# ugonfor/DGQ

Hardware: AMD Instinct MI355X
Metric: UNet denoise steps/sec @ SD1.4 512^2 W4A8 g16 (higher is better)
Workload: dtype int8 (W4A8 MFMA, int32 accumulate; fp32 between layers); 1 GPU; SD v1.4 UNet W4A8 g=16 (time-aware, log2 softmax real-time δ, start-peak), DDIM 50-step schedule, 512x512 (64x64 latents), CFG pair per step per GPU; config_id=c2, prompts_per_gpu=1, batch_per_gpu=2, parallelism=replicas x1 (no collectives)

## Files before the change

### dgq_amd/_lib.py

```python
import ctypes
import os

import torch

_HERE = os.path.dirname(os.path.abspath(__file__))
LIB_PATH = os.environ.get("DGQ_HIP_LIB") or os.path.join(_HERE, "csrc", "libdgq_hip.so")

_vp, _i, _f, _i64 = ctypes.c_void_p, ctypes.c_int, ctypes.c_float, ctypes.c_int64
ABI_VERSION = 123

SIGNATURES = {
    "dgq_version": [],
    "dgq_quantize_weight": [_vp, _vp, _vp, _vp, _i, _i, _i, _vp, _vp],
    "dgq_pack_w4": [_vp, _i, _i, _vp, _i, _i, _vp, _vp],
    "dgq_unpack_w4": [_vp, _i, _i, _i, _vp, _vp],
    "dgq_pack_w8": [_vp, _i, _i, _vp, _i, _vp, _vp],
    "dgq_quant_act": [_vp, _i, _i, _i, _i, _i, _i, _i, _i, _i, _vp, _vp, _vp, _i, _i, _vp, _vp, _i, _i, _vp, _vp, _i,
                      _vp, _vp, _i, _vp, _vp, _f, _vp],
    "dgq_groupnorm_scale_shift": [_vp, _i, _i, _i, _i, _i, _f, _vp, _vp, _vp, _vp, _vp, _i, _vp],
    "dgq_quant_act_parts": [_i, _i],
    "dgq_gemm_wxa8": [_vp, _vp, _i, _i, _i, _vp, _i, _i, _i, _vp, _vp, _vp, _vp, _i, _f, _vp, _vp, _vp, _vp, _vp, _i, _i,
                      _vp, ctypes.c_size_t, _vp, _vp],
    "dgq_gemm_workspace_bytes": [_i, _i, _i],
    "dgq_gemm_plan_splits": [_i, _i, _i, _i, _i, ctypes.c_size_t],
    "dgq_gemm_act_fuses": [_i, _i, _i, _i, _i, _i, _i, _i, _i],
    "dgq_gemm_conv_act_fuses": [_i] * 14,
    "dgq_groupnorm_from_partials": [_vp, _i, _vp, _i, _i, _i, _i, _f, _vp, _vp, _vp, _vp, _vp],
    "dgq_fakequant_rows": [_vp, _vp, _i, _i, _i, _i, _i, _i, _vp, _vp, _i, _i, _vp],
    "dgq_max_f32": [_vp, _i64, _i, _i, _vp, _vp],
    "dgq_logquant_f32": [_vp, _vp, _i64, _i, _i, _vp, _i, _vp],
    "dgq_attention_f32": [_vp, _vp, _vp, _vp, _i, _i, _i, _i, _i, _f, _i, _i, _vp, _i, _vp, _vp, ctypes.c_size_t, _vp],
    "dgq_attention": [_vp, _vp, _vp, _vp, _i, _i, _i, _i, _i, _i, _f, _i, _i, _vp, _i, _vp, _vp, ctypes.c_size_t, _vp],
    "dgq_conv2d_f32w": [_vp, _i, _i, _i, _i, _i, _i, _i, _i, _i, _vp, _vp, _i, _vp, _i, _i, _vp, _vp, _i, _vp, _i, _vp, _vp],
    "dgq_conv2d_wq": [_vp, _i, _i, _i, _i, _i, _i, _i, _i, _i, _i, _vp, _i, _i, _vp, _vp, _vp, _i, _i, _vp, _i, _i, _vp],
    "dgq_attention_fuses_fakequant": [_i, _i],
    "dgq_attention_workspace_bytes": [_i, _i, _i, _i, _i],
    "dgq_attention_sync_timeouts": [],
    "dgq_minmax_rows_cols": [_vp, _i, _i, _i, _i64, _vp, _vp, _vp, _vp, _vp, _i, _vp],
    "dgq_linear_smallm_batch": [_vp, _i, _i, _i, _i64, _i, _i, _vp, _i, _vp],
    "dgq_quant_act_batch": [_i, _vp, _vp],
    "dgq_quant_act_variant": [_vp],
    "dgq_quant_act_conv_tile": [_i, _i, _i, _i, _i, _vp],
    "dgq_gemm_wxa8_batch": [_i, _vp, _vp],
    "dgq_adaround_soft_fwd": [_vp, _vp, _vp, _vp, _i, _i, _i, _vp, _vp],
    "dgq_adaround_soft_bwd": [_vp, _vp, _vp, _vp, _vp, _i, _i, _i, _vp, _vp],
    "dgq_adaround_reg_blocks": [_i64],
    "dgq_adaround_reg_fwd": [_vp, _i64, _f, _vp, _vp],
    "dgq_adaround_reg_bwd": [_vp, _i64, _f, _vp, _vp, _vp],
    "dgq_timestep_embedding": [_vp, _i, _i64, _i, _i, _vp, _i, _vp],
    "dgq_cfg_ddim_step": [_vp, _vp, _vp, _vp, _i, _i64, _i, _i, _i, _f, _f, _f, _f, _f, _vp],
}



class GemmExtra(ctypes.Structure):
    _fields_ = [("residual", _vp), ("ldr", _i), ("res_div", _i), ("res_dtype", _i), ("fq_mode", _i), ("fq_delta", _vp), ("fq_zp", _vp),
                ("fq_T", _i), ("fq_D", _i), ("fq_skip", _i), ("fq_qmax", _f), ("geglu", _i), ("gn_partial", _vp), ("conv", _vp), ("flush_coef", _vp), ("wfrag", _vp), ("act", _vp), ("y2", _vp), ("ldy2", _i)]


class GemmAct(ctypes.Structure):
    _fields_ = [("x", _vp), ("x_dtype", _i), ("ldx", _i), ("K", _i), ("kdst", _vp), ("czp", _vp), ("bits", _i),
                ("pre_scale", _vp), ("pre_shift", _vp), ("rows_per_image", _i), ("pre_act", _i),
                ("ln_gamma", _vp), ("ln_beta", _vp), ("ln_eps", _f),
                ("kpat", _vp), ("B", _i), ("H", _i), ("W", _i), ("kh", _i), ("kw", _i), ("stride", _i), ("pad", _i)]


class GemmConv(ctypes.Structure):
    _fields_ = [("codes_in", _vp), ("pixsum", _vp), ("fill", _vp), ("B", _i), ("H", _i), ("W", _i), ("C", _i), ("ldc", _i), ("kh", _i),
                ("kw", _i), ("stride", _i), ("pad", _i), ("Ho", _i), ("Wo", _i), ("zero_code", _f), ("pixsum_parts", _i)]


class SmallMProblem(ctypes.Structure):
    _fields_ = [("wpacked", _vp), ("alpha", _vp), ("zw", _vp), ("gamma", _vp), ("vn", _vp), ("mdelta", _vp), ("mzp", _vp),
                ("y", _vp), ("ldy", _i), ("N", _i), ("Kp", _i), ("w_bits", _i), ("a_bits", _i)]


class QuantActArgs(ctypes.Structure):
    _fields_ = [("x", _vp), ("x_dtype", _i), ("B", _i), ("H", _i), ("W", _i), ("C", _i), ("kh", _i), ("kw", _i), ("stride", _i),
                ("pad", _i), ("ksrc", _vp), ("koff", _vp), ("klds", _vp), ("kdst", _vp), ("Kp", _i), ("per_m", _i), ("delta", _vp), ("zp", _vp),
                ("L", _i), ("bits", _i), ("codes", _vp), ("rowsum", _vp), ("ksplits", _i), ("pre_scale", _vp), ("pre_shift", _vp),
                ("pre_act", _i), ("ln_gamma", _vp), ("ln_beta", _vp), ("ln_eps", _f), ("kpat", _vp), ("ups", _i)]


class GemmArgs(ctypes.Structure):
    _fields_ = [("codes", _vp), ("rowsum", _vp), ("rowsum_parts", _i), ("M", _i), ("Kp", _i), ("wpacked", _vp), ("w_bits", _i),
                ("N", _i), ("per_m", _i), ("cdelta", _vp), ("cflush", _vp), ("mdelta", _vp), ("mzp", _vp), ("L", _i),
                ("offset", _f), ("alpha", _vp), ("zw", _vp), ("gamma", _vp), ("vn", _vp), ("y", _vp), ("y_dtype", _i), ("ldy", _i),
                ("extra", _vp)]


class AttnFq(ctypes.Structure):
    _fields_ = [("mode", _i), ("skip", _i), ("bits", _i), ("delta", _vp), ("zero_point", _vp)]


_lib = None


def load():
    global _lib
    if _lib is None:
        if not os.path.exists(LIB_PATH):
            raise RuntimeError(
                "dgq_amd: %s not found — build it with `make -C dgq_amd/csrc` (or __graft_entry__.build()); "
                "there is no CPU fallback" % LIB_PATH)
        lib = ctypes.CDLL(LIB_PATH)
        for name, args in SIGNATURES.items():
            fn = getattr(lib, name)
            fn.argtypes = args
            fn.restype = ctypes.c_size_t if name.endswith("_workspace_bytes") else ctypes.c_int
        if lib.dgq_version() != ABI_VERSION:
            raise RuntimeError("dgq_amd: %s is ABI revision %d, this binding was written against %d (include/dgq_hip.h: "
                               "DGQ_ABI_VERSION) — rebuild with `make -C dgq_amd/csrc`" % (LIB_PATH, lib.dgq_version(), ABI_VERSION))
        lib.dgq_last_error.argtypes = []
        lib.dgq_last_error.restype = ctypes.c_char_p
        _lib = lib
    return _lib


def last_error():
    return load().dgq_last_error().decode()


def check(rc, what):
    if rc != 0:
        raise RuntimeError("%s failed (%d): %s" % (what, rc, last_error()))


DTYPE_CODE = {torch.float32: 0, torch.float16: 1, torch.bfloat16: 2}


def ptr(t):
    if t is None:
        return None
    assert t.is_cuda, "dgq_amd kernels need device tensors (no CPU path)"
    return ctypes.c_void_p(t.data_ptr())


def stream():
    return ctypes.c_void_p(torch.cuda.current_stream().cuda_stream)


def require_gpu():
    if not torch.cuda.is_available():
        raise RuntimeError("dgq_amd: no GPU visible — the quantized path runs only through the HIP kernels "
                           "(no CPU fallback)")
    load()
```

### dgq_amd/csrc/attn_bf16x3.hip

```cpp
#include "attn_bf16x3_dev.h"

DGQ_DIAG_BUFFER(attn)


template <int D, typename TIn, int QM, bool VINT>
__global__ __launch_bounds__(256) void attn3_prep_kernel(const TIn* __restrict__ k, const TIn* __restrict__ v,
                                                         unsigned char* __restrict__ planes, int B, int H, int S, int NT,
                                                         FqDesc fk, FqDesc fv, float* __restrict__ delta_reset, int n_reset,
                                                         const TIn* __restrict__ q, float* __restrict__ qfq, int T, FqDesc fqq) {
    using G = Geo<D, QM, VINT>;
    constexpr bool QI8 = QM == 1;
    static_assert(D % 8 == 0, "head_dim must be a multiple of 8");
    const int bh = blockIdx.y, b = bh / H, hd = bh - b * H;
    DGQ_DIAG_DECL
    DGQ_STAMP(0); DGQ_STAMP_REAL(1); DGQ_STAMP_WHERE(2);
#ifdef DGQ_DIAG
    dg.t[13] = 1;
#define DGQ_ATTN_PREP_DONE() do { DGQ_STAMP(9); DGQ_DIAG_DRAIN(); DGQ_STAMP(10); DGQ_STAMP_REAL(11); DGQ_DIAG_FLUSH(attn, 4, (threadIdx.x >> 6) + 32768, threadIdx.x & 63); } while (0)
#else
#define DGQ_ATTN_PREP_DONE() do {} while (0)
#endif
    if (QM == 2 && (int)blockIdx.x >= 2 * NT) {
        const int t0 = ((int)blockIdx.x - 2 * NT) * 32;
        constexpr int QC = D / 8;
        unsigned short* qb = reinterpret_cast<unsigned short*>(qfq);
        float* qtab = reinterpret_cast<float*>(qb + (size_t)B * T * H * D);
        const float off = 0.5f * (fqq.qmax + 1.0f);
        constexpr int QIT = (32 * QC + 255) / 256;
        float x[QIT][8];
#pragma unroll
        for (int it = 0; it < QIT; ++it) {
            const int i = threadIdx.x + 256 * it, r = i / QC, c8 = i - r * QC;
            if (i < 32 * QC && t0 + r < T) load8<TIn>(q + ((int64_t)(b * T + t0 + r) * H + hd) * D + 8 * c8, x[it]);
        }
#pragma unroll
        for (int it = 0; it < QIT; ++it) {
            const int i = threadIdx.x + 256 * it, r = i / QC, c8 = i - r * QC;
            const int t = t0 + r;
            if (i >= 32 * QC || t >= T) continue;
            const int64_t row = (int64_t)(b * T + t) * H + hd;
            unsigned w[4];
#pragma unroll
            for (int j = 0; j < 8; ++j) {
                const int idx = fqq.mode == 0 ? 0 : (fqq.mode == 1 ? t - fqq.skip : 8 * c8 + j);
                const float dl = fqq.delta[idx];
                const unsigned bits = bf16_bits(fq_code(x[it][j], dl, dgq_rcp(dl), fqq.zp[idx], fqq.qmax, off));
                if (j & 1) w[j >> 1] |= bits << 16; else w[j >> 1] = bits;
            }
            *reinterpret_cast<uint4*>(qb + row * D + 8 * c8) = make_uint4(w[0], w[1], w[2], w[3]);
            if (c8 == 0) {
                const int idx = fqq.mode == 0 ? 0 : t - fqq.skip;
                qtab[row * 2] = fqq.mode == 2 ? 1.0f : fqq.delta[idx];
                qtab[row * 2 + 1] = fqq.mode == 2 ? 1.0f : fqq.zp[idx] - off;
            }
        }
        DGQ_ATTN_PREP_DONE(); return;
    }
    if (QI8 && (int)blockIdx.x >= 2 * NT) {
        const int t = ((int)blockIdx.x - 2 * NT) * 32 + (threadIdx.x >> 3);
        const int part = threadIdx.x & 7;
        int8_t* qc = reinterpret_cast<int8_t*>(qfq);
        float* qtab = reinterpret_cast<float*>(reinterpret_cast<unsigned char*>(qfq) + (size_t)B * T * H * G::DP32);
        if (t < T) {
            const int64_t row = (int64_t)(b * T + t) * H + hd;
            const int idx = fqq.mode == 0 ? 0 : t - fqq.skip;
            const float dl = fqq.delta[idx], z = fqq.zp[idx], inv = dgq_rcp(dl);
            const float off = 0.5f * (fqq.qmax + 1.0f);
            const float zc = z - off;
            const TIn* k0 = k + ((int64_t)(b * S) * H + hd) * D;
            float csum = 0.0f, sp = 0.0f;
            for (int c8 = part; c8 < G::DP32 / 8; c8 += 8) {
                float x[8] = {0.f, 0.f, 0.f, 0.f, 0.f, 0.f, 0.f, 0.f};
                unsigned w0 = 0, w1 = 0;
                if (8 * c8 < D) {
                    load8<TIn>(q + row * D + 8 * c8, x);
                    float kk[8] = {0.f, 0.f, 0.f, 0.f, 0.f, 0.f, 0.f, 0.f};
                    if (fk.skip > 0) load8<TIn>(k0 + 8 * c8, kk);
#pragma unroll
                    for (int j = 0; j < 8; ++j) {
                        const float c = fq_code(x[j], dl, inv, z, fqq.qmax, off);
                        csum += c;
                        sp += (c - zc) * kk[j];
                        const unsigned byte = ((unsigned)(int)c) & 0xFFu;
                        if (j < 4) w0 |= byte << (8 * j); else w1 |= byte << (8 * (j - 4));
                    }
                }
                *reinterpret_cast<uint2*>(qc + row * G::DP32 + 8 * c8) = make_uint2(w0, w1);
            }
#pragma unroll
            for (int o = 4; o > 0; o >>= 1) {
                csum += __shfl_xor(csum, o, 64);
                sp += __shfl_xor(sp, o, 64);
            }
            if (part == 0) *reinterpret_cast<float4*>(qtab + row * 4) = make_float4(dl, zc, csum - (float)D * zc, sp);
        }
        DGQ_ATTN_PREP_DONE(); return;
    }
    if ((int)blockIdx.x >= 2 * NT) {
        const int t0 = ((int)blockIdx.x - 2 * NT) * 32;
        constexpr int QC = D / 8;
        for (int i = threadIdx.x; i < 32 * QC; i += 256) {
            const int r = i / QC, c8 = i - r * QC;
            const int t = t0 + r;
            if (t >= T) continue;
            const int64_t o = ((int64_t)(b * T + t) * H + hd) * D + 8 * c8;
            float x[8];
            load8<TIn>(q + o, x);
            fq_apply8(fqq, x, t, 8 * c8);
            *reinterpret_cast<float4*>(qfq + o) = make_float4(x[0], x[1], x[2], x[3]);
            *reinterpret_cast<float4*>(qfq + o + 4) = make_float4(x[4], x[5], x[6], x[7]);
        }
        DGQ_ATTN_PREP_DONE(); return;
    }
    const bool do_k = (int)blockIdx.x < NT;
    const int tile = do_k ? (int)blockIdx.x : (int)blockIdx.x - NT;
    const int s0 = tile * KT;
    if (delta_reset && blockIdx.x == 0 && bh == 0)
        for (int i = threadIdx.x; i < n_reset; i += 256) delta_reset[i] = 0.0f;
    const int64_t kbase = ((int64_t)(b * S) * H + hd) * D, vbase = kbase;
    const int64_t HD = (int64_t)H * D;
    unsigned short* kimg = reinterpret_cast<unsigned short*>(planes + ((int64_t)bh * NT + tile) * G::IMG_BYTES);
    unsigned short* vimg = kimg + G::K_ELEMS;
    const TypedLd<TIn> ld{};
    if (do_k) prep_k_tile<D, QM, VINT>(ld, k, kbase, HD, S, s0, fk, fqq, kimg, threadIdx.x);
    else prep_v_tile<D, QM, VINT>(ld, v, vbase, HD, S, s0, fv, vimg, threadIdx.x);
    DGQ_ATTN_PREP_DONE();
}

template <int D, int NW, int QM, int TPS = 1>
__global__ __launch_bounds__(64 * NW) void attn3_stats_kernel(AttnParams p) {
    using G = Geo<D, QM>;
    constexpr bool QI8 = G::QI8, KS = QM == 3;
    constexpr int ST = TPS > 1 ? 3 : G::STATS_STAGES, NP = G::K_PIECES, TB = NP * 1024, SB = TPS * TB;
    extern __shared__ __attribute__((aligned(16))) unsigned char lds8[];
    const int tid = threadIdx.x, lane = tid & 63, wid = tid >> 6, h32 = lane >> 5;
    DGQ_DIAG_DECL
    DGQ_STAMP(0); DGQ_STAMP_REAL(1); DGQ_STAMP_WHERE(2);
#ifdef DGQ_DIAG
    dg.t[13] = 2;
#endif
    int bx, bh;
    attn_block_coords(p.xcd, bx, bh);
    const int b = bh / p.H, hd = bh - b * p.H;
    const int t = bx * (32 * NW) + wid * 32 + (lane & 31);
    const int tq = min(t, p.T - 1);
    const unsigned char* img_lane = p.planes + (int64_t)bh * p.NT * p.img_bytes + lane * 16;
    const uint32_t lds_base = (uint32_t)(uintptr_t)(lptr_t)lds8;
    const int nsp = gridDim.z, i0 = (int)((long)p.NT * blockIdx.z / nsp), i1 = (int)((long)p.NT * (blockIdx.z + 1) / nsp);
#pragma unroll
    for (int i = 0; i < ST - 1; ++i)
#pragma unroll
        for (int j = 0; j < TPS; ++j)
            issue_image<NP, NW>(img_lane + (int64_t)min(i0 + TPS * i + j, i1 - 1) * p.img_bytes, lds_base + i * SB + j * TB, wid);
    bf16x8 qf[3][QI8 ? 1 : G::NKK];
    v4i qc[G::NK32];
    float4 qt = make_float4(1.0f, 0.0f, 0.0f, 0.0f);
    if constexpr (QI8) load_q_i8<D>(qc, qt, p, (int64_t)(b * p.T + tq) * p.H + hd, h32);
    else if constexpr (QM == 2) load_q1<D>(qf, reinterpret_cast<const unsigned short*>(p.q) + ((int64_t)(b * p.T + tq) * p.H + hd) * D, h32);
    else load_q<D>(qf, p.q + ((int64_t)(b * p.T + tq) * p.H + hd) * D, h32, p.fq[0], tq);
    if constexpr (QM == 2) {
        const float2 t2 = *reinterpret_cast<const float2*>(p.qtab + ((int64_t)(b * p.T + tq) * p.H + hd) * 2);
        qt.x = t2.x;
        qt.y = t2.y;
        if constexpr (G::FOLDZ) fold_zmul<D>(qf, qt.y, h32);
    }
    float inv_dk = 1.0f, cq = 0.0f, dk = 1.0f;
    if constexpr (KS) {
        dk = p.fq[1].delta[0];
        inv_dk = 1.0f / dk;
        cq = -(p.fq[1].zp[0] - 0.5f * (p.fq[1].qmax + 1.0f)) * qt.z;
    }
    const float sl2 = p.scale * LOG2E * qt.x * dk;
    float mraw = -INFINITY, l = 0.0f, m2raw = -INFINITY;
    DGQ_STAMP(3);
    wait_image<NP, TPS * (ST - 2), NW>(wid);
    __builtin_amdgcn_s_barrier();
    DGQ_STAMP(4);
    int stage = 0, istage = ST - 1;
    for (int ib = i0; ib < i1; ib += TPS) {
#pragma unroll
      for (int jt = 0; jt < TPS; ++jt)
        issue_image<NP, NW>(img_lane + (int64_t)min(ib + TPS * (ST - 1) + jt, i1 - 1) * p.img_bytes, lds_base + istage * SB + jt * TB, wid);
#pragma unroll
      for (int jt = 0; jt < TPS; ++jt) {
        const int i = ib + jt;
        const unsigned char* tile_lds = lds8 + stage * SB + jt * TB;
        const int s0 = i * KT;
        v16f acc;
        if constexpr (QI8) acc = score_tile_i8<D, KS>(tile_lds, qc, qt, lane, i == 0 && p.kskip > 0, inv_dk, cq);
        else if constexpr (QM == 2) acc = score_tile_q1<D>(reinterpret_cast<const unsigned short*>(tile_lds), qf, qt.y, lane);
        else acc = score_tile<D>(reinterpret_cast<const unsigned short*>(tile_lds), qf, lane);
        const bool edge = (s0 + KT > p.S) || (s0 < p.skip);
        float tmax = -INFINITY, tmax2 = -INFINITY;
        if (edge) {
#pragma unroll
            for (int r = 0; r < 16; ++r) {
                const int s = s0 + key_of(r, h32);
                if (s >= p.S) acc[r] = -INFINITY;
                tmax = fmaxf(tmax, acc[r]);
                if (s >= p.skip) tmax2 = fmaxf(tmax2, acc[r]);
            }
        } else {
#pragma unroll
            for (int r = 0; r < 16; ++r) tmax = fmaxf(tmax, acc[r]);
            tmax2 = tmax;
        }
        const float mn = fmaxf(mraw, tmax);
        const float nb = (mn == -INFINITY) ? 0.0f : -(mn * sl2);
        f2 part = {0.0f, 0.0f};
        const f2 sl2v = {sl2, sl2}, nbv = {nb, nb};
#pragma unroll
        for (int r = 0; r < 16; r += 2) {
            const f2 a = pk_fma(f2{acc[r], acc[r + 1]}, sl2v, nbv);
            part = pk_add(part, f2{__builtin_amdgcn_exp2f(a.x), __builtin_amdgcn_exp2f(a.y)});
        }
        l = l * __builtin_amdgcn_exp2f(fmaf(mraw, sl2, nb)) + (part.x + part.y);
        mraw = mn;
        m2raw = fmaxf(m2raw, tmax2);
      }
        wait_image<NP, TPS * (ST - 2), NW>(wid);
        __builtin_amdgcn_s_barrier();
        stage = (stage + 1 == ST) ? 0 : stage + 1;
        istage = (istage + 1 == ST) ? 0 : istage + 1;
    }
    asm volatile("s_waitcnt vmcnt(0)" ::: "memory");
    DGQ_STAMP(5);
    {
        const float mo = __shfl_xor(mraw, 32, 64), lo = __shfl_xor(l, 32, 64);
        const float mm = fmaxf(mraw, mo), nb = -(mm * sl2);
        l = l * __builtin_amdgcn_exp2f(fmaf(mraw, sl2, nb)) + lo * __builtin_amdgcn_exp2f(fmaf(mo, sl2, nb));
        mraw = mm;
        m2raw = fmaxf(m2raw, __shfl_xor(m2raw, 32, 64));
    }
    mraw += cq;
    m2raw += cq;
    const float m = mraw * sl2;
    if (nsp > 1) {
        if (t < p.T && h32 == 0)
            *reinterpret_cast<float4*>(p.stats_part + (((int64_t)blockIdx.z * p.B * p.H + bh) * p.T + t) * 4) = make_float4(m, l, m2raw * sl2, 0.0f);
        DGQ_STAMP(9); DGQ_DIAG_DRAIN(); DGQ_STAMP(10); DGQ_STAMP_REAL(11);
        DGQ_DIAG_FLUSH(attn, NW, wid + 16384, lane);
        return;
    }
    if (t < p.T && h32 == 0) {
        float* st = p.stats + ((int64_t)bh * p.T + t) * 2;
        st[0] = m;
        st[1] = l;
    }
    if (p.mode == 1) {
        float pm = (t < p.T) ? exp2f(m2raw * sl2 - m) / l : 0.0f;
#pragma unroll
        for (int o = 32; o > 0; o >>= 1) pm = fmaxf(pm, __shfl_xor(pm, o, 64));
        float* wmax = reinterpret_cast<float*>(lds8);
        __syncthreads();
        if (lane == 0) wmax[wid] = pm;
        __syncthreads();
        if (tid == 0) {
#pragma unroll
            for (int w = 1; w < NW; ++w) pm = fmaxf(pm, wmax[w]);
            const int slot = (blockIdx.x + gridDim.x * blockIdx.y) & (DELTA_SLOTS - 1);
            atomicMax(reinterpret_cast<int*>(p.delta) + slot, __float_as_int(pm));
        }
    }
    DGQ_STAMP(9); DGQ_DIAG_DRAIN(); DGQ_STAMP(10); DGQ_STAMP_REAL(11);
    DGQ_DIAG_FLUSH(attn, NW, wid + 16384, lane);
}

template <typename T>
__global__ __launch_bounds__(256) void attn3_add16_kernel(T* __restrict__ o, const float* __restrict__ part0, const float* __restrict__ part1, int64_t n4) {
    const int64_t i = (int64_t)blockIdx.x * 256 + threadIdx.x;
    if (i < n4) {
        const float4 a = reinterpret_cast<const float4*>(part0)[i], c = reinterpret_cast<const float4*>(part1)[i];
        T t[4] = {dgq_from_float<T>(a.x + c.x), dgq_from_float<T>(a.y + c.y), dgq_from_float<T>(a.z + c.z), dgq_from_float<T>(a.w + c.w)};
        reinterpret_cast<uint2*>(o)[i] = *reinterpret_cast<const uint2*>(t);
    }
}

__global__ __launch_bounds__(256) void attn3_add_kernel(float* __restrict__ o, const float* __restrict__ part, int64_t n4) {
    const int64_t i = (int64_t)blockIdx.x * 256 + threadIdx.x;
    if (i < n4) {
        float4 a = reinterpret_cast<float4*>(o)[i];
        const float4 c = reinterpret_cast<const float4*>(part)[i];
        a.x += c.x; a.y += c.y; a.z += c.z; a.w += c.w;
        reinterpret_cast<float4*>(o)[i] = a;
    }
}

__global__ __launch_bounds__(256) void attn3_merge_kernel(AttnParams p) {
    const int64_t row = (int64_t)blockIdx.x * 256 + threadIdx.x, rows = (int64_t)p.B * p.H * p.T;
    float pm = 0.0f;
    if (row < rows) {
        const float4 a = *reinterpret_cast<const float4*>(p.stats_part + row * 4);
        const float4 c = *reinterpret_cast<const float4*>(p.stats_part + (rows + row) * 4);
        const float m = fmaxf(a.x, c.x);
        const float l = a.y * exp2f(a.x - m) + c.y * exp2f(c.x - m);
        p.stats[row * 2] = m;
        p.stats[row * 2 + 1] = l;
        if (p.mode == 1) pm = exp2f(fmaxf(a.z, c.z) - m) / l;
    }
    if (p.mode == 1) {
#pragma unroll
        for (int o = 32; o > 0; o >>= 1) pm = fmaxf(pm, __shfl_xor(pm, o, 64));
        __shared__ float wmax[4];
        if ((threadIdx.x & 63) == 0) wmax[threadIdx.x >> 6] = pm;
        __syncthreads();
        if (threadIdx.x == 0) {
            pm = fmaxf(fmaxf(wmax[0], wmax[1]), fmaxf(wmax[2], wmax[3]));
            atomicMax(reinterpret_cast<int*>(p.delta) + (blockIdx.x & (DELTA_SLOTS - 1)), __float_as_int(pm));
        }
    }
}

template <int D, bool UNIFORM, int NW, int QM, bool VINT, int TPS = 1>
__global__ __launch_bounds__(64 * NW) void attn3_pv_kernel(AttnParams p) {
    using G = Geo<D, QM, VINT>;
    constexpr bool QI8 = G::QI8, KS = QM == 3;
    constexpr int ST = TPS > 1 ? 2 : G::PV_STAGES, NP = G::IMG_PIECES, TB = G::IMG_BYTES, SB = TPS * TB;
    extern __shared__ __attribute__((aligned(16))) unsigned char lds8[];
    const int tid = threadIdx.x, lane = tid & 63, wid = tid >> 6, h32 = lane >> 5;
    DGQ_DIAG_DECL
    DGQ_STAMP(0); DGQ_STAMP_REAL(1); DGQ_STAMP_WHERE(2);
#ifdef DGQ_DIAG
    dg.t[13] = 3;
#endif
    int bx, bh;
    attn_block_coords(p.xcd, bx, bh);
    const int b = bh / p.H, hd = bh - b * p.H;
    const int t = bx * (32 * NW) + wid * 32 + (lane & 31);
    const int tq = min(t, p.T - 1);
    const unsigned char* img_lane = p.planes + (int64_t)bh * p.NT * G::IMG_BYTES + lane * 16;
    const uint32_t lds_base = (uint32_t)(uintptr_t)(lptr_t)lds8;
    const int nsp = gridDim.z, i0 = (int)((long)p.NT * blockIdx.z / nsp), i1 = (int)((long)p.NT * (blockIdx.z + 1) / nsp);
#pragma unroll
    for (int i = 0; i < ST - 1; ++i)
#pragma unroll
        for (int j = 0; j < TPS; ++j)
            issue_image<NP, NW>(img_lane + (int64_t)min(i0 + TPS * i + j, i1 - 1) * G::IMG_BYTES, lds_base + i * SB + j * TB, wid);
    bf16x8 qf[3][QI8 ? 1 : G::NKK];
    v4i qc[G::NK32];
    float4 qt = make_float4(1.0f, 0.0f, 0.0f, 0.0f);
    if constexpr (QI8) load_q_i8<D>(qc, qt, p, (int64_t)(b * p.T + tq) * p.H + hd, h32);
    else if constexpr (QM == 2) load_q1<D>(qf, reinterpret_cast<const unsigned short*>(p.q) + ((int64_t)(b * p.T + tq) * p.H + hd) * D, h32);
    else load_q<D>(qf, p.q + ((int64_t)(b * p.T + tq) * p.H + hd) * D, h32, p.fq[0], tq);
    if constexpr (QM == 2) {
        const float2 t2 = *reinterpret_cast<const float2*>(p.qtab + ((int64_t)(b * p.T + tq) * p.H + hd) * 2);
        qt.x = t2.x;
        qt.y = t2.y;
        if constexpr (G::FOLDZ) fold_zmul<D>(qf, qt.y, h32);
    }
    float inv_dk = 1.0f, cq = 0.0f, dk = 1.0f;
    if constexpr (KS) {
        dk = p.fq[1].delta[0];
        inv_dk = 1.0f / dk;
        cq = -(p.fq[1].zp[0] - 0.5f * (p.fq[1].qmax + 1.0f)) * qt.z;
    }
    const float2 ml = *reinterpret_cast<const float2*>(p.stats + ((int64_t)bh * p.T + tq) * 2);
    const float l = ml.y;
    float delta;
    if (p.mode == 1) {
        delta = p.delta[lane];
#pragma unroll
        for (int o = 32; o > 0; o >>= 1) delta = fmaxf(delta, __shfl_xor(delta, o, 64));
    } else {
        delta = p.delta[0];
    }
    const float sl2 = p.scale * LOG2E * qt.x * dk;
    const float nsl2 = -sl2;
    const float m = ml.x - cq * sl2;
    const float a0 = m + log2f(l) + log2f(delta);
    const float inv_l = 1.0f / l;
    constexpr float MAGIC = 12582912.0f;
    constexpr int MAGIC_I = 0x4B400000;
    const int cmax_i = MAGIC_I + min((int)p.qmax, 127);
    float p_bypass = 0.0f;
    float psum = 0.0f;
    v16f oacc[G::NDT];
#pragma unroll
    for (int j = 0; j < G::NDT; ++j)
#pragma unroll
        for (int r = 0; r < 16; ++r) oacc[j][r] = 0.0f;
    constexpr int VPL = G::DV * G::VLD;
    DGQ_STAMP(3);
    asm volatile("s_waitcnt vmcnt(0)" ::: "memory");
    __builtin_amdgcn_s_barrier();
    DGQ_STAMP(4);
    int stage = 0, istage = ST - 1;
    for (int ib = i0; ib < i1; ib += TPS) {
#pragma unroll
      for (int jt = 0; jt < TPS; ++jt)
        issue_image<NP, NW>(img_lane + (int64_t)min(ib + TPS * (ST - 1) + jt, i1 - 1) * G::IMG_BYTES, lds_base + istage * SB + jt * TB, wid);
#pragma unroll
      for (int jt = 0; jt < TPS; ++jt) {
        const int i = ib + jt;
        const int s0 = i * KT;
        const unsigned short* kbc = reinterpret_cast<const unsigned short*>(lds8 + stage * SB + jt * TB);
        const unsigned short* vtc = kbc + G::K_ELEMS;
        v16f acc;
        if constexpr (QI8) acc = score_tile_i8<D, KS>(lds8 + stage * SB + jt * TB, qc, qt, lane, i == 0 && p.kskip > 0, inv_dk, cq);
        else if constexpr (QM == 2) acc = score_tile_q1<D>(kbc, qf, qt.y, lane);
        else acc = score_tile<D>(kbc, qf, lane);
        const bool edge = (s0 + KT > p.S) || (s0 < p.skip);
        auto quantise = [&](auto edge_tag) {
            constexpr bool EDGE = decltype(edge_tag)::value;
#pragma unroll
            for (int r = 0; r < 16; ++r) {
                float ph;
                if (UNIFORM) {
                    const float pr = exp2f(fmaf(acc[r], sl2, -m)) * inv_l;
                    ph = fminf(fmaxf(rintf(__fdiv_rn(pr, delta)), 0.0f), p.qmax);
                } else {
                    const float x = fmaf(acc[r], nsl2, a0);
                    int ci = __float_as_int(x + MAGIC);
                    ci = min(max(ci, MAGIC_I), cmax_i);
                    ph = __int_as_float(0x3F800000 - (ci << 23));
                }
                if (EDGE) {
                    const int s = s0 + key_of(r, h32);
                    if (s >= p.S) ph = 0.0f;
                    else if (s < p.skip) {
                        p_bypass = exp2f(fmaf(acc[r], sl2, -m)) * inv_l;
                        ph = 0.0f;
                    }
                }
                acc[r] = ph;
                if constexpr (VINT && !G::VONES) psum += ph;
            }
        };
        bf16x8 pf[2];
        if (UNIFORM && !edge) {
            const int cmaxu_i = MAGIC_I + (int)p.qmax;
            const f2 sl2v = {sl2, sl2}, na0v = {-a0, -a0}, magic = {MAGIC, MAGIC}, nmagic = {-MAGIC, -MAGIC};
            f2 ps2 = {0.0f, 0.0f};
            unsigned w[8];
#pragma unroll
            for (int r = 0; r < 16; r += 2) {
                const f2 a = pk_fma(f2{acc[r], acc[r + 1]}, sl2v, na0v);
                const f2 y = pk_add(f2{__builtin_amdgcn_exp2f(a.x), __builtin_amdgcn_exp2f(a.y)}, magic);
                const f2 c = pk_add(f2{__int_as_float(min(__float_as_int(y.x), cmaxu_i)), __int_as_float(min(__float_as_int(y.y), cmaxu_i))}, nmagic);
                if constexpr (VINT && !G::VONES) ps2 = pk_add(ps2, c);
                w[r >> 1] = __builtin_amdgcn_perm(__float_as_uint(c.y), __float_as_uint(c.x), 0x07060302u);
            }
            if constexpr (VINT && !G::VONES) psum += ps2.x + ps2.y;
            pf[0] = __builtin_bit_cast(bf16x8, make_uint4(w[0], w[1], w[2], w[3]));
            pf[1] = __builtin_bit_cast(bf16x8, make_uint4(w[4], w[5], w[6], w[7]));
        } else if (!UNIFORM && !edge) {
            int ci[16];
            const f2 nsl2v = {nsl2, nsl2}, a0m = {a0, a0}, magic = {MAGIC, MAGIC};
#pragma unroll
            for (int r = 0; r < 16; r += 2) {
                const f2 y = pk_add(pk_fma(f2{acc[r], acc[r + 1]}, nsl2v, a0m), magic);
                ci[r] = min(max(__float_as_int(y.x), MAGIC_I), cmax_i);
                ci[r + 1] = min(max(__float_as_int(y.y), MAGIC_I), cmax_i);
                if constexpr (VINT && !G::VONES) psum += __int_as_float(0x3F800000 - (ci[r] << 23)) + __int_as_float(0x3F800000 - (ci[r + 1] << 23));
            }
#pragma unroll
            for (int ks = 0; ks < 2; ++ks) {
                unsigned w[4];
#pragma unroll
                for (int i = 0; i < 4; ++i) {
                    const unsigned pair = __builtin_amdgcn_perm((unsigned)ci[8 * ks + 2 * i + 1], (unsigned)ci[8 * ks + 2 * i], 0x05040100u);
                    w[i] = (unsigned)(__mul24((int)pair, -128) + 0x3F803F80);
                }
                pf[ks] = __builtin_bit_cast(bf16x8, make_uint4(w[0], w[1], w[2], w[3]));
            }
        } else {
            if (edge) quantise(std::true_type{});
            else quantise(std::false_type{});
#pragma unroll
            for (int ks = 0; ks < 2; ++ks) {
#define PK(i) ((__float_as_uint(acc[8 * ks + 2 * (i)]) >> 16) | (__float_as_uint(acc[8 * ks + 2 * (i) + 1]) & 0xFFFF0000u))
                pf[ks] = __builtin_bit_cast(bf16x8, make_uint4(PK(0), PK(1), PK(2), PK(3)));
#undef PK
            }
        }
#pragma unroll
        for (int j = 0; j < G::NDT; ++j) {
            const unsigned short* vp = vtc + (j * 32 + (lane & 31)) * G::VLD + 8 * h32;
#pragma unroll
            for (int ks = 0; ks < 2; ++ks) {
                const bf16x8 vh = *reinterpret_cast<const bf16x8*>(vp + 16 * ks);
                if constexpr (!VINT) {
                    const bf16x8 vm = *reinterpret_cast<const bf16x8*>(vp + VPL + 16 * ks);
                    const bf16x8 vl = *reinterpret_cast<const bf16x8*>(vp + 2 * VPL + 16 * ks);
                    oacc[j] = __builtin_amdgcn_mfma_f32_32x32x16_bf16(vl, pf[ks], oacc[j], 0, 0, 0);
                    oacc[j] = __builtin_amdgcn_mfma_f32_32x32x16_bf16(vm, pf[ks], oacc[j], 0, 0, 0);
                }
                oacc[j] = __builtin_amdgcn_mfma_f32_32x32x16_bf16(vh, pf[ks], oacc[j], 0, 0, 0);
            }
        }
      }
        wait_image<NP, TPS * (ST - 2), NW>(wid);
        __builtin_amdgcn_s_barrier();
        stage = (stage + 1 == ST) ? 0 : stage + 1;
        istage = (istage + 1 == ST) ? 0 : istage + 1;
    }
    asm volatile("s_waitcnt vmcnt(0)" ::: "memory");
    DGQ_STAMP(5);
    if (p.skip > 0) p_bypass = __shfl(p_bypass, lane & 31, 64);
    if constexpr (G::VONES) {
        constexpr int kd = D % 32, rr = (kd & 3) + 4 * (kd >> 3), hh = (kd >> 2) & 1;
        psum = __shfl(oacc[D / 32][rr], (lane & 31) + 32 * hh, 64);
    } else if (VINT) {
        psum += __shfl_xor(psum, 32, 64);
    }
    float* vtab = reinterpret_cast<float*>(lds8);
    __syncthreads();
    for (int d = tid; d < G::DV; d += 64 * NW) {
        float t0 = 1.0f, t1 = 0.0f, t2 = 0.0f;
        if (VINT) {
            const int idx = (p.fq[2].mode == 0 || d >= D) ? 0 : d;
            t0 = p.fq[2].delta[idx];
            t1 = p.fq[2].zp[idx] - 0.5f * (p.fq[2].qmax + 1.0f);
        }
        if (p.skip > 0 && d < D) t2 = fq_apply(p.fq[2], load_any(p.v, p.io_dtype, ((int64_t)(b * p.S) * p.H + hd) * D + d), 0, d);
        vtab[d] = t0; vtab[G::DV + d] = t1; vtab[2 * G::DV + d] = t2;
    }
    __syncthreads();
    DGQ_STAMP(6);
    {
        constexpr int ELD = 36;
        float* ep = reinterpret_cast<float*>(lds8) + 3 * G::DV + wid * (32 * ELD);
        const int tw0 = bx * (32 * NW) + wid * 32;
        const int er = lane >> 3, ec = (lane & 7) * 4;
        float* const fpart = blockIdx.z > 0 ? p.o_part : ((gridDim.z > 1 && p.io_dtype != DGQ_F32) ? p.o_part0 : nullptr);
        const float pb = p.skip > 0 ? p_bypass : 0.0f;
#pragma unroll
        for (int j = 0; j < G::NDT; ++j) {
            DGQ_STAMP_NOW(dg_e0);
            float4 t0[4], t1[4], t2[4];
#pragma unroll
            for (int k4 = 0; k4 < 4; ++k4) {
                const int d = j * 32 + 8 * k4 + 4 * h32;
                t0[k4] = *reinterpret_cast<const float4*>(vtab + d);
                t1[k4] = *reinterpret_cast<const float4*>(vtab + G::DV + d);
                t2[k4] = *reinterpret_cast<const float4*>(vtab + 2 * G::DV + d);
            }
#pragma unroll
            for (int k4 = 0; k4 < 4; ++k4) {
                const float a0[4] = {t0[k4].x, t0[k4].y, t0[k4].z, t0[k4].w}, a1[4] = {t1[k4].x, t1[k4].y, t1[k4].z, t1[k4].w};
                const float a2[4] = {t2[k4].x, t2[k4].y, t2[k4].z, t2[k4].w};
                float o4[4];
#pragma unroll
                for (int e = 0; e < 4; ++e) {
                    const int r = 4 * k4 + e;
                    float o;
                    if (VINT) o = delta * (a0[e] * (oacc[j][r] - a1[e] * psum));
                    else o = delta * oacc[j][r];
                    o4[e] = o + pb * a2[e];
                }
                *reinterpret_cast<float4*>(ep + (lane & 31) * ELD + 8 * k4 + 4 * h32) = make_float4(o4[0], o4[1], o4[2], o4[3]);
            }
            DGQ_STAMP_ACC(7, dg_e0);
            DGQ_STAMP_NOW(dg_e1);
            float4 ov[4];
#pragma unroll
            for (int ps = 0; ps < 4; ++ps) ov[ps] = *reinterpret_cast<const float4*>(ep + (er + 8 * ps) * ELD + ec);
#pragma unroll
            for (int ps = 0; ps < 4; ++ps) {
                const int row = er + 8 * ps, tt = tw0 + row, d0 = j * 32 + ec;
                const float4 v = ov[ps];
                if (tt < p.T && d0 < D) {
                    const int64_t oi = ((int64_t)(b * p.T + tt) * p.H + hd) * D + d0;
                    if (fpart) {
                        *reinterpret_cast<float4*>(fpart + oi) = v;
                    } else if (p.io_dtype == DGQ_F32) {
                        *reinterpret_cast<float4*>(reinterpret_cast<float*>(p.o) + oi) = v;
                    } else if (p.io_dtype == DGQ_F16) {
                        __half hv[4] = {__float2half(v.x), __float2half(v.y), __float2half(v.z), __float2half(v.w)};
                        *reinterpret_cast<uint2*>(reinterpret_cast<__half*>(p.o) + oi) = *reinterpret_cast<const uint2*>(hv);
                    } else {
                        __hip_bfloat16 hv[4] = {__float2bfloat16(v.x), __float2bfloat16(v.y), __float2bfloat16(v.z), __float2bfloat16(v.w)};
                        *reinterpret_cast<uint2*>(reinterpret_cast<__hip_bfloat16*>(p.o) + oi) = *reinterpret_cast<const uint2*>(hv);
                    }
                }
            }
            DGQ_STAMP_ACC(12, dg_e1);
        }
    }
    DGQ_STAMP(9); DGQ_DIAG_DRAIN(); DGQ_STAMP(10); DGQ_STAMP_REAL(11);
    DGQ_DIAG_FLUSH(attn, NW, wid, lane);
}

template <int D, int QM, bool VINT>
static int launch_attn3(AttnParams p, const void* q_raw, unsigned char* planes, float* qfq, hipStream_t st) {
    using G = Geo<D, QM, VINT>;
    constexpr bool QI8 = G::QI8;
    constexpr int PQM = QM == 3 ? 1 : QM;
    p.planes = planes;
    p.img_bytes = G::IMG_BYTES;
    constexpr int stats_lds = G::STATS_STAGES * G::K_PIECES * 1024;
    constexpr int TPS_S = (3 * DGQ_ATTN_TPS_STATS * G::K_PIECES * 1024 <= 160 * 1024) ? DGQ_ATTN_TPS_STATS : 2;
    constexpr int stats2_lds = D <= 64 ? 3 * TPS_S * G::K_PIECES * 1024 : 0;
    constexpr int pv_ring = G::PV_STAGES * G::IMG_BYTES, pv_scratch = 3 * G::DV * 4 + 8 * 32 * 36 * 4;
    constexpr int pv_lds = pv_ring > pv_scratch ? pv_ring : pv_scratch;
    constexpr int TPS_P = (2 * DGQ_ATTN_TPS_PV * G::IMG_BYTES <= 160 * 1024) ? DGQ_ATTN_TPS_PV : 2;
    constexpr int pv2_ring = D <= 64 ? 2 * TPS_P * G::IMG_BYTES : 0, pv2_lds = pv2_ring > pv_scratch ? pv2_ring : pv_scratch;
    static_assert(stats_lds <= 160 * 1024 && pv_lds <= 160 * 1024 && stats2_lds <= 160 * 1024 && pv2_lds <= 160 * 1024, "LDS ring too large");
    static std::atomic<bool> attr_set[64];
    int dev = 0;
    (void)hipGetDevice(&dev);
    if (dev < 0 || dev >= 64 || !attr_set[dev].load(std::memory_order_acquire)) {
        (void)hipFuncSetAttribute(reinterpret_cast<const void*>(&attn3_stats_kernel<D, 4, QM>), hipFuncAttributeMaxDynamicSharedMemorySize, stats_lds);
        (void)hipFuncSetAttribute(reinterpret_cast<const void*>(&attn3_pv_kernel<D, true, 4, QM, VINT>), hipFuncAttributeMaxDynamicSharedMemorySize, pv_lds);
        (void)hipFuncSetAttribute(reinterpret_cast<const void*>(&attn3_pv_kernel<D, false, 4, QM, VINT>), hipFuncAttributeMaxDynamicSharedMemorySize, pv_lds);
        if constexpr (D <= 64) {
            (void)hipFuncSetAttribute(reinterpret_cast<const void*>(&attn3_stats_kernel<D, 8, QM>), hipFuncAttributeMaxDynamicSharedMemorySize, stats_lds);
            (void)hipFuncSetAttribute(reinterpret_cast<const void*>(&attn3_stats_kernel<D, 8, QM, TPS_S>), hipFuncAttributeMaxDynamicSharedMemorySize, stats2_lds);
            (void)hipFuncSetAttribute(reinterpret_cast<const void*>(&attn3_pv_kernel<D, true, 8, QM, VINT>), hipFuncAttributeMaxDynamicSharedMemorySize, pv_lds);
            (void)hipFuncSetAttribute(reinterpret_cast<const void*>(&attn3_pv_kernel<D, false, 8, QM, VINT>), hipFuncAttributeMaxDynamicSharedMemorySize, pv_lds);
            (void)hipFuncSetAttribute(reinterpret_cast<const void*>(&attn3_pv_kernel<D, true, 8, QM, VINT, TPS_P>), hipFuncAttributeMaxDynamicSharedMemorySize, pv2_lds);
            (void)hipFuncSetAttribute(reinterpret_cast<const void*>(&attn3_pv_kernel<D, false, 8, QM, VINT, TPS_P>), hipFuncAttributeMaxDynamicSharedMemorySize, pv2_lds);
        }
        if (dev >= 0 && dev < 64) attr_set[dev].store(true, std::memory_order_release);
    }
    const bool q_copy = QM != 0 || ((p.fq[0].mode >= 0 || p.io_dtype != DGQ_F32) && qfq != nullptr);
    const dim3 pgrid(2 * p.NT + (q_copy ? (p.T + 31) / 32 : 0), p.B * p.H);
    float* dreset = p.mode == 1 ? p.delta : nullptr;
    const long one_wgs = (long)((p.T + 127) / 128) * p.B * p.H;
    const int n_reset = DELTA_SLOTS + ((p.NT <= 8 && one_wgs <= DELTA_GRANULES) ? (512 - 4 * DELTA_SLOTS) / 4 + 2 * (int)one_wgs : 0);
#define DGQ_PREP(TT) hipLaunchKernelGGL((attn3_prep_kernel<D, TT, PQM, VINT>), pgrid, dim3(256), 0, st, (const TT*)p.k, (const TT*)p.v, planes, \
                                        p.B, p.H, p.S, p.NT, p.fq[1], p.fq[2], dreset, n_reset, (const TT*)q_raw, qfq, p.T, p.fq[0])
    if (p.io_dtype == DGQ_F16) DGQ_PREP(__half);
    else if (p.io_dtype == DGQ_BF16) DGQ_PREP(__hip_bfloat16);
    else DGQ_PREP(float);
#undef DGQ_PREP
    p.kskip = 0;
    p.qcodes = nullptr;
    p.qtab = nullptr;
    if (QI8) {
        p.qcodes = reinterpret_cast<const int8_t*>(qfq);
        p.qtab = reinterpret_cast<const float*>(reinterpret_cast<const unsigned char*>(qfq) + (size_t)p.B * p.T * p.H * G::DP32);
        p.kskip = p.fq[1].skip;
        p.q = nullptr;
        p.fq[0].mode = -1;
    } else if (QM == 2) {
        p.q = qfq;
        p.qtab = reinterpret_cast<const float*>(reinterpret_cast<const unsigned short*>(qfq) + (size_t)p.B * p.T * p.H * D);
        p.fq[0].mode = -1;
    } else if (q_copy) {
        p.q = qfq;
        p.fq[0].mode = -1;
    } else {
        p.q = reinterpret_cast<const float*>(q_raw);
    }
    {
        const int one = dgq_attention_one_launch(p, D, QM, VINT, p.mode == 1 ? reinterpret_cast<unsigned*>(p.delta) + 128 : nullptr, st);
        if (one <= 0) return one;
    }
    const long nblk8 = (long)((p.T + 255) / 256) * p.B * p.H;
    const long rounds8 = (nblk8 + 511) / 512;
    const bool tail_ok = nblk8 <= 512 || 10 * nblk8 >= 8 * 512 * rounds8;
    const bool wide = D <= 64 && nblk8 >= 256 && tail_ok;
    const char* se = getenv("DGQ_ATTN_SPLIT");
    const long split_below = se ? atol(se) : 448L;
    const long nblk4 = (long)((p.T + 127) / 128) * p.B * p.H;
    const int nsp = (!wide && nblk4 < split_below && p.NT >= 8 && D % 4 == 0) ? 2 : 1;
    if (wide) {
        if constexpr (D <= 64) {
            dim3 grid((p.T + 255) / 256, p.B * p.H), block(512);
            if (p.NT >= 4 * TPS_S && p.NT % TPS_S == 0) hipLaunchKernelGGL((attn3_stats_kernel<D, 8, QM, TPS_S>), grid, block, stats2_lds, st, p);
            else hipLaunchKernelGGL((attn3_stats_kernel<D, 8, QM>), grid, block, stats_lds, st, p);
            if (p.NT >= 4 * TPS_P && p.NT % TPS_P == 0) {
                if (p.mode == 3) hipLaunchKernelGGL((attn3_pv_kernel<D, true, 8, QM, VINT, TPS_P>), grid, block, pv2_lds, st, p);
                else hipLaunchKernelGGL((attn3_pv_kernel<D, false, 8, QM, VINT, TPS_P>), grid, block, pv2_lds, st, p);
            } else if (p.mode == 3) hipLaunchKernelGGL((attn3_pv_kernel<D, true, 8, QM, VINT>), grid, block, pv_lds, st, p);
            else hipLaunchKernelGGL((attn3_pv_kernel<D, false, 8, QM, VINT>), grid, block, pv_lds, st, p);
        }
    } else {
        dim3 grid((p.T + 127) / 128, p.B * p.H, nsp), block(256);
        hipLaunchKernelGGL((attn3_stats_kernel<D, 4, QM>), grid, block, stats_lds, st, p);
        if (nsp > 1) hipLaunchKernelGGL(attn3_merge_kernel, dim3((unsigned)(((long)p.B * p.H * p.T + 255) / 256)), dim3(256), 0, st, p);
        if (p.mode == 3) hipLaunchKernelGGL((attn3_pv_kernel<D, true, 4, QM, VINT>), grid, block, pv_lds, st, p);
        else hipLaunchKernelGGL((attn3_pv_kernel<D, false, 4, QM, VINT>), grid, block, pv_lds, st, p);
    }
    if (nsp > 1) {
        const int64_t n4 = (int64_t)p.B * p.T * p.H * D / 4;
        const dim3 ag((unsigned)((n4 + 255) / 256));
        if (p.io_dtype == DGQ_F32) hipLaunchKernelGGL(attn3_add_kernel, ag, dim3(256), 0, st, reinterpret_cast<float*>(p.o), p.o_part, n4);
        else if (p.io_dtype == DGQ_BF16) hipLaunchKernelGGL(attn3_add16_kernel<__hip_bfloat16>, ag, dim3(256), 0, st, reinterpret_cast<__hip_bfloat16*>(p.o), p.o_part0, p.o_part, n4);
        else hipLaunchKernelGGL(attn3_add16_kernel<__half>, ag, dim3(256), 0, st, reinterpret_cast<__half*>(p.o), p.o_part0, p.o_part, n4);
    }
    return dgq_launch_status("dgq_attention_f32(bf16x3)");
}

size_t dgq_attention_qi8_bytes(int B, int H, int T, int D) {
    const size_t dp32 = (size_t)(D + 31) / 32 * 32;
    const size_t i8 = (size_t)B * T * H * (dp32 + 16), q1 = (size_t)B * T * H * (D + 2) * sizeof(float);
    return i8 > q1 ? i8 : q1;
}

size_t dgq_attention_bf16x3_bytes(int B, int H, int S, int D) {
    const size_t NT = (size_t)(S + KT - 1) / KT;
    size_t img;
#define DGQ_IMG(DD) case DD: img = Geo<DD, 2, false>::IMG_BYTES > Geo<DD, 0, false>::IMG_BYTES ? Geo<DD, 2, false>::IMG_BYTES : Geo<DD, 0, false>::IMG_BYTES; break
    switch (D) {
        DGQ_IMG(8);
        DGQ_IMG(16);
        DGQ_IMG(40);
        DGQ_IMG(64);
        DGQ_IMG(80);
        DGQ_IMG(160);
        default: return 0;
    }
#undef DGQ_IMG
    return (size_t)B * H * NT * img;
}

int dgq_attention_bf16x3(const void* q, const void* k, const void* v, void* o, int io_dtype, int B, int H, int T, int S, int D,
                         float scale, int mode, int skip, float qmax, float* stats_ws, float* delta_ws, void* planes,
                         float* qfq, float* o_part, const dgq_attn_fq_t* fq, hipStream_t st) {
    AttnParams p;
    p.stats_part = stats_ws + (((size_t)B * H * T * 2 + 3) & ~(size_t)3);
    p.o_part = o_part;
    p.o_part0 = o_part + (((size_t)B * T * H * D * sizeof(float) + 255) / 256 * 256) / sizeof(float);
    for (int i = 0; i < 3; ++i) {
        p.fq[i].mode = -1; p.fq[i].skip = 0; p.fq[i].qmax = 0.0f; p.fq[i].delta = nullptr; p.fq[i].zp = nullptr;
        if (fq && fq[i].mode >= 0) {
            p.fq[i].mode = fq[i].mode; p.fq[i].skip = fq[i].skip; p.fq[i].qmax = (float)((1 << fq[i].bits) - 1);
            p.fq[i].delta = fq[i].delta; p.fq[i].zp = fq[i].zero_point;
        }
    }
    p.q = nullptr; p.k = k; p.v = v; p.o = o; p.io_dtype = io_dtype; p.B = B; p.H = H; p.T = T; p.S = S; p.scale = scale;
    p.mode = mode; p.skip = skip;
    p.qmax = qmax; p.stats = stats_ws; p.delta = delta_ws;
    p.NT = (S + KT - 1) / KT;
    p.xcd = 1;
    p.qcodes = nullptr; p.qtab = nullptr; p.kskip = 0;
    unsigned char* img = reinterpret_cast<unsigned char*>(planes);
    const char* i8_env = getenv("DGQ_ATTN_I8");
    const bool i8_off = i8_env != nullptr && i8_env[0] == '0';
    const bool qi8 = !i8_off && qfq != nullptr && p.fq[0].mode >= 0 && p.fq[0].mode <= 1 && p.fq[1].mode >= 0 && p.fq[1].mode <= 1 &&
                     p.fq[0].skip == 0;
    const int qm = qi8 ? 1 : ((!i8_off && qfq != nullptr && p.fq[0].mode >= 0 && p.fq[0].skip == 0) ? 2 : 0);
    const bool kscalar = qi8 && p.fq[1].mode == 0;
    const bool vint = !i8_off && (p.fq[2].mode == 0 || p.fq[2].mode == 2);
#define DGQ_ATTN_V(DD, QQ) (vint ? launch_attn3<DD, QQ, true>(p, q, img, qfq, st) : launch_attn3<DD, QQ, false>(p, q, img, qfq, st))
#define DGQ_ATTN_CASE(DD) case DD: return qm == 1 ? (kscalar ? DGQ_ATTN_V(DD, 3) : DGQ_ATTN_V(DD, 1)) : (qm == 2 ? DGQ_ATTN_V(DD, 2) : DGQ_ATTN_V(DD, 0))
    switch (D) {
        DGQ_ATTN_CASE(8);
        DGQ_ATTN_CASE(16);
        DGQ_ATTN_CASE(40);
        DGQ_ATTN_CASE(64);
        DGQ_ATTN_CASE(80);
        DGQ_ATTN_CASE(160);
        default: return 1;
    }
#undef DGQ_ATTN_CASE
#undef DGQ_ATTN_V
}
```

### dgq_amd/csrc/attn_bf16x3_dev.h

```cpp
#pragma once
#include <atomic>
#include <type_traits>
#include "dgq_common.h"
#include "diag.h"

typedef float v16f __attribute__((ext_vector_type(16)));
typedef int v16i __attribute__((ext_vector_type(16)));
typedef __bf16 bf16x8 __attribute__((ext_vector_type(8)));

#define KT 32
#ifndef DGQ_ATTN_TPS_STATS
#define DGQ_ATTN_TPS_STATS 2
#endif
#ifndef DGQ_ATTN_TPS_PV
#define DGQ_ATTN_TPS_PV 2
#endif
#ifndef DGQ_PV_ST64
#define DGQ_PV_ST64 2
#endif
#define DELTA_SLOTS 64
#define DELTA_GRANULES 1024
#define DELTA_AREA_BYTES (512 + 8 * DELTA_GRANULES)
typedef float f2 __attribute__((ext_vector_type(2)));
#ifndef DGQ_ATTN_PK
#define DGQ_ATTN_PK 1
#endif
#if DGQ_ATTN_PK
__device__ __forceinline__ f2 pk_fma(f2 a, f2 b, f2 c) { return __builtin_elementwise_fma(a, b, c); }
__device__ __forceinline__ f2 pk_mul(f2 a, f2 b) { return a * b; }
__device__ __forceinline__ f2 pk_add(f2 a, f2 b) { return a + b; }
#else
__device__ __forceinline__ f2 pk_fma(f2 a, f2 b, f2 c) { return f2{fmaf(a.x, b.x, c.x), fmaf(a.y, b.y, c.y)}; }
__device__ __forceinline__ f2 pk_mul(f2 a, f2 b) { return f2{a.x * b.x, a.y * b.y}; }
__device__ __forceinline__ f2 pk_add(f2 a, f2 b) { return f2{a.x + b.x, a.y + b.y}; }
#endif
#define LOG2E 1.4426950408889634f

struct FqDesc {
    int mode;
    int skip;
    float qmax;
    const float* delta;
    const float* zp;
};

__device__ __forceinline__ float fq_apply(const FqDesc& f, float x, int t, int d) {
    if (f.mode < 0 || t < f.skip) return x;
    const int idx = f.mode == 0 ? 0 : (f.mode == 1 ? t - f.skip : d);
    const float dl = f.delta[idx], z = f.zp[idx];
    return dl * (dgq_affine_code_fast(x, dl, dgq_rcp(dl), z, f.qmax) - z);
}

__device__ __forceinline__ void fq_apply8(const FqDesc& f, float (&x)[8], int t, int d0) {
    if (f.mode < 0 || t < f.skip) return;
    if (f.mode == 2) {
        const float4 da = *reinterpret_cast<const float4*>(f.delta + d0), db = *reinterpret_cast<const float4*>(f.delta + d0 + 4);
        const float4 za = *reinterpret_cast<const float4*>(f.zp + d0), zb = *reinterpret_cast<const float4*>(f.zp + d0 + 4);
        const float dl[8] = {da.x, da.y, da.z, da.w, db.x, db.y, db.z, db.w};
        const float zz[8] = {za.x, za.y, za.z, za.w, zb.x, zb.y, zb.z, zb.w};
#pragma unroll
        for (int j = 0; j < 8; ++j) x[j] = dl[j] * (dgq_affine_code_fast(x[j], dl[j], dgq_rcp(dl[j]), zz[j], f.qmax) - zz[j]);
    } else {
        const int idx = f.mode == 0 ? 0 : t - f.skip;
        const float dl = f.delta[idx], z = f.zp[idx], inv = dgq_rcp(dl);
#pragma unroll
        for (int j = 0; j < 8; ++j) x[j] = dl * (dgq_affine_code_fast(x[j], dl, inv, z, f.qmax) - z);
    }
}

struct AttnParams {
    FqDesc fq[3];
    const float* q;
    const void* k;
    const void* v;
    void* o;
    int io_dtype;
    int B, H, T, S;
    float scale;
    int mode;
    int skip;
    float qmax;
    float* stats;
    float* stats_part;
    float* o_part;
    float* o_part0;
    float* delta;
    const unsigned char* planes;
    int NT;
    const int8_t* qcodes;
    const float* qtab;
    int img_bytes;
    int kskip;
    int xcd;
};

__device__ __forceinline__ unsigned short bf16_bits(float x) {
    return __builtin_bit_cast(unsigned short, __float2bfloat16(x));
}
__device__ __forceinline__ float bf16_to_f(unsigned short b) { return __uint_as_float(((unsigned)b) << 16); }

__device__ __forceinline__ void split3(float x, unsigned short& h, unsigned short& m, unsigned short& l) {
    h = bf16_bits(x);
    const float r1 = x - bf16_to_f(h);
    m = bf16_bits(r1);
    const float r2 = r1 - bf16_to_f(m);
    l = bf16_bits(r2);
}

template <typename TIn> __device__ __forceinline__ void load8(const TIn* p, float (&x)[8]);
template <> __device__ __forceinline__ void load8<float>(const float* p, float (&x)[8]) {
    const float4 a = *reinterpret_cast<const float4*>(p), c = *reinterpret_cast<const float4*>(p + 4);
    x[0] = a.x; x[1] = a.y; x[2] = a.z; x[3] = a.w; x[4] = c.x; x[5] = c.y; x[6] = c.z; x[7] = c.w;
}
template <> __device__ __forceinline__ void load8<__half>(const __half* p, float (&x)[8]) {
    const uint4 t = *reinterpret_cast<const uint4*>(p);
    const __half* h = reinterpret_cast<const __half*>(&t);
#pragma unroll
    for (int j = 0; j < 8; ++j) x[j] = __half2float(h[j]);
}
template <> __device__ __forceinline__ void load8<__hip_bfloat16>(const __hip_bfloat16* p, float (&x)[8]) {
    const uint4 t = *reinterpret_cast<const uint4*>(p);
    const unsigned short* h = reinterpret_cast<const unsigned short*>(&t);
#pragma unroll
    for (int j = 0; j < 8; ++j) x[j] = __uint_as_float(((unsigned)h[j]) << 16);
}
__device__ __forceinline__ float load_any(const void* p, int dtype, int64_t i) {
    if (dtype == DGQ_F16) return __half2float(reinterpret_cast<const __half*>(p)[i]);
    if (dtype == DGQ_BF16) return __bfloat162float(reinterpret_cast<const __hip_bfloat16*>(p)[i]);
    return reinterpret_cast<const float*>(p)[i];
}
__device__ __forceinline__ void store_any(void* p, int dtype, int64_t i, float v) {
    if (dtype == DGQ_F16) reinterpret_cast<__half*>(p)[i] = __float2half(v);
    else if (dtype == DGQ_BF16) reinterpret_cast<__hip_bfloat16*>(p)[i] = __float2bfloat16(v);
    else reinterpret_cast<float*>(p)[i] = v;
}

template <int D, int QM = 0, bool VINT = false> struct Geo {
    static constexpr bool QI8 = QM == 1 || QM == 3;
    static constexpr int DP = (D + 15) / 16 * 16;
    static constexpr int NKK = DP / 16;
    static constexpr int NDT = (D + 31) / 32;
    static constexpr int DV = NDT * 32;
    static constexpr int KLD = DP + 8;
    static constexpr int VLD = KT + 8;
    static constexpr int DP32 = (D + 31) / 32 * 32;
    static constexpr int NK32 = DP32 / 32;
    static constexpr int K8_LD = DP32 + 16;
    static constexpr int K8_BYTES = KT * K8_LD;
    static constexpr int KTAB_BYTES = 3 * KT * 4;
    static constexpr int K_ELEMS = QI8 ? (K8_BYTES + KTAB_BYTES) / 2 : 3 * KT * KLD + (QM == 2 ? 2 * KT : 0);
    static constexpr int V_PLANES = VINT ? 1 : 3;
    static constexpr bool FOLDZ = QM == 2 && (DP - D) >= 3;
    static constexpr bool VONES = VINT && (NDT * 32 > D);
    static constexpr int V_ELEMS = V_PLANES * DV * VLD;
    static constexpr int K_PIECES = (2 * K_ELEMS + 1023) / 1024;
    static constexpr int IMG_PIECES = (2 * (K_ELEMS + V_ELEMS) + 1023) / 1024;
    static constexpr int IMG_BYTES = IMG_PIECES * 1024;
    static constexpr int STATS_STAGES = D <= 80 ? 4 : 3;
    static constexpr int PV_STAGES = D == 64 ? (IMG_BYTES <= 16 * 1024 ? DGQ_PV_ST64 : 2) : ((D <= 40 || D == 80) ? 3 : 2);
};

template <int D> using GeoI8 = Geo<D, 1, false>;

typedef __attribute__((address_space(3))) void* lptr_t;

__device__ __forceinline__ void glds16(const void* gsrc, uint32_t lds_addr) {
    asm volatile("s_nop 0\n\tglobal_load_lds_dwordx4 %0, off" : : "v"(gsrc), "{m0}"(lds_addr) : "memory");
}

template <int NP, int NW>
__device__ __forceinline__ void issue_image(const unsigned char* img_lane, uint32_t lds_stage, int wid) {
#pragma unroll
    for (int i = 0; i < (NP + NW - 1) / NW; ++i) {
        const int j = wid + NW * i;
        if (j < NP) glds16(img_lane + 1024 * j, __builtin_amdgcn_readfirstlane(lds_stage + 1024 * j));
    }
}

template <int NP, int YOUNGER, int NW>
__device__ __forceinline__ void wait_image(int wid) {
    constexpr int HI = (NP + NW - 1) / NW, LO = NP / NW;
    static_assert(HI * YOUNGER <= 63, "vmcnt immediate");
    if (HI == LO || wid < NP % NW) asm volatile("s_waitcnt vmcnt(%0)" ::"n"(HI * YOUNGER) : "memory");
    else asm volatile("s_waitcnt vmcnt(%0)" ::"n"(LO * YOUNGER) : "memory");
}

__device__ __forceinline__ float fq_code(float x, float dl, float inv, float z, float qmax, float off) {
    return dgq_affine_code_fast(x, dl, inv, z, qmax) - off;
}


template <int D>
__device__ __forceinline__ void load_q(bf16x8 (&qf)[3][Geo<D>::NKK], const float* qrow, int h32, const FqDesc& fq, int t) {
    using G = Geo<D>;
#pragma unroll
    for (int kk = 0; kk < G::NKK; ++kk) {
        const int d0 = 16 * kk + 8 * h32;
        float x[8] = {0.0f, 0.0f, 0.0f, 0.0f, 0.0f, 0.0f, 0.0f, 0.0f};
        if (d0 < D) {
            const float4 a = *reinterpret_cast<const float4*>(qrow + d0), c = *reinterpret_cast<const float4*>(qrow + d0 + 4);
            x[0] = a.x; x[1] = a.y; x[2] = a.z; x[3] = a.w; x[4] = c.x; x[5] = c.y; x[6] = c.z; x[7] = c.w;
            fq_apply8(fq, x, t, d0);
        }
        unsigned wh[4], wm[4], wl[4];
#pragma unroll
        for (int j = 0; j < 4; ++j) {
            unsigned short h0, m0, l0, h1, m1, l1;
            split3(x[2 * j], h0, m0, l0);
            split3(x[2 * j + 1], h1, m1, l1);
            wh[j] = (unsigned)h0 | ((unsigned)h1 << 16);
            wm[j] = (unsigned)m0 | ((unsigned)m1 << 16);
            wl[j] = (unsigned)l0 | ((unsigned)l1 << 16);
        }
        qf[0][kk] = __builtin_bit_cast(bf16x8, make_uint4(wh[0], wh[1], wh[2], wh[3]));
        qf[1][kk] = __builtin_bit_cast(bf16x8, make_uint4(wm[0], wm[1], wm[2], wm[3]));
        qf[2][kk] = __builtin_bit_cast(bf16x8, make_uint4(wl[0], wl[1], wl[2], wl[3]));
    }
}

template <int D>
__device__ __forceinline__ v16f score_tile(const unsigned short* kb, const bf16x8 (&qf)[3][Geo<D>::NKK], int lane) {
    using G = Geo<D>;
    constexpr bool DUAL = D >= 64;
    v16f acc, acc2;
#pragma unroll
    for (int r = 0; r < 16; ++r) acc[r] = acc2[r] = 0.0f;
    const unsigned short* kp = kb + (lane & 31) * G::KLD + 8 * (lane >> 5);
    constexpr int PL = KT * G::KLD;
#pragma unroll
    for (int kk = 0; kk < G::NKK; ++kk) {
        const bf16x8 kh = *reinterpret_cast<const bf16x8*>(kp + 16 * kk);
        const bf16x8 km = *reinterpret_cast<const bf16x8*>(kp + PL + 16 * kk);
        const bf16x8 kl = *reinterpret_cast<const bf16x8*>(kp + 2 * PL + 16 * kk);
        if (DUAL) {
            acc2 = __builtin_amdgcn_mfma_f32_32x32x16_bf16(kl, qf[0][kk], acc2, 0, 0, 0);
            acc = __builtin_amdgcn_mfma_f32_32x32x16_bf16(km, qf[0][kk], acc, 0, 0, 0);
            acc2 = __builtin_amdgcn_mfma_f32_32x32x16_bf16(kh, qf[2][kk], acc2, 0, 0, 0);
            acc = __builtin_amdgcn_mfma_f32_32x32x16_bf16(kh, qf[1][kk], acc, 0, 0, 0);
            acc2 = __builtin_amdgcn_mfma_f32_32x32x16_bf16(km, qf[1][kk], acc2, 0, 0, 0);
            acc = __builtin_amdgcn_mfma_f32_32x32x16_bf16(kh, qf[0][kk], acc, 0, 0, 0);
        } else {
            acc = __builtin_amdgcn_mfma_f32_32x32x16_bf16(kl, qf[0][kk], acc, 0, 0, 0);
            acc = __builtin_amdgcn_mfma_f32_32x32x16_bf16(kh, qf[2][kk], acc, 0, 0, 0);
            acc = __builtin_amdgcn_mfma_f32_32x32x16_bf16(km, qf[1][kk], acc, 0, 0, 0);
            acc = __builtin_amdgcn_mfma_f32_32x32x16_bf16(km, qf[0][kk], acc, 0, 0, 0);
            acc = __builtin_amdgcn_mfma_f32_32x32x16_bf16(kh, qf[1][kk], acc, 0, 0, 0);
            acc = __builtin_amdgcn_mfma_f32_32x32x16_bf16(kh, qf[0][kk], acc, 0, 0, 0);
        }
    }
    if (DUAL) {
#pragma unroll
        for (int r = 0; r < 16; ++r) acc[r] += acc2[r];
    }
    return acc;
}

__device__ __forceinline__ int key_of(int r, int h) { return (r & 3) + 8 * (r >> 2) + 4 * h; }

template <int D>
__device__ __forceinline__ void load_q_i8(v4i (&qc)[GeoI8<D>::NK32], float4& qt, const AttnParams& p, int64_t row, int h32) {
    using G = Geo<D, true>;
    const int8_t* src = p.qcodes + row * G::DP32 + 16 * h32;
#pragma unroll
    for (int kk = 0; kk < G::NK32; ++kk) qc[kk] = *reinterpret_cast<const v4i*>(src + 32 * kk);
    qt = *reinterpret_cast<const float4*>(p.qtab + row * 4);
}

template <int D, bool KS>
__device__ __forceinline__ v16f score_tile_i8(const unsigned char* kimg, const v4i (&qc)[GeoI8<D>::NK32], const float4& qt,
                                              int lane, bool bypass_key0, float inv_dk, float cq) {
    using G = Geo<D, true>;
    v16i acc;
#pragma unroll
    for (int r = 0; r < 16; ++r) acc[r] = 0;
    const unsigned char* kp = kimg + (lane & 31) * G::K8_LD + 16 * (lane >> 5);
#pragma unroll
    for (int kk = 0; kk < G::NK32; ++kk) {
        const v4i kf = *reinterpret_cast<const v4i*>(kp + 32 * kk);
        acc = __builtin_amdgcn_mfma_i32_32x32x32_i8(kf, qc[kk], acc, 0, 0, 0);
    }
    const float* ktab = reinterpret_cast<const float*>(kimg + G::K8_BYTES);
    const int h32 = lane >> 5;
    const f2 zq = {qt.y, qt.y}, zs = {qt.z, qt.z};
    v16f out;
#pragma unroll
    for (int g = 0; g < 4; ++g) {
        const float4 ns = *reinterpret_cast<const float4*>(ktab + 2 * KT + 8 * g + 4 * h32);
        float4 dk, nz;
        if constexpr (!KS) {
            dk = *reinterpret_cast<const float4*>(ktab + 8 * g + 4 * h32);
            nz = *reinterpret_cast<const float4*>(ktab + KT + 8 * g + 4 * h32);
        }
#pragma unroll
        for (int e = 0; e < 4; e += 2) {
            const f2 a = {(float)acc[4 * g + e], (float)acc[4 * g + e + 1]};
            f2 v = pk_fma(zq, e ? f2{ns.z, ns.w} : f2{ns.x, ns.y}, a);
            if constexpr (!KS) {
                v = pk_fma(zs, e ? f2{nz.z, nz.w} : f2{nz.x, nz.y}, v);
                v = pk_mul(v, e ? f2{dk.z, dk.w} : f2{dk.x, dk.y});
            }
            out[4 * g + e] = v.x;
            out[4 * g + e + 1] = v.y;
        }
    }
    if (bypass_key0 && h32 == 0) out[0] = KS ? fmaf(qt.w, inv_dk, -cq) : qt.w;
    return out;
}

template <int D>
__device__ __forceinline__ void load_q1(bf16x8 (&qf)[3][Geo<D>::NKK], const unsigned short* qrow, int h32) {
#pragma unroll
    for (int kk = 0; kk < Geo<D>::NKK; ++kk) {
        const int d0 = 16 * kk + 8 * h32;
        qf[0][kk] = d0 < D ? *reinterpret_cast<const bf16x8*>(qrow + d0) : __builtin_bit_cast(bf16x8, make_uint4(0u, 0u, 0u, 0u));
    }
}

template <int D>
__device__ __forceinline__ void fold_zmul(bf16x8 (&qf)[3][Geo<D>::NKK], float zmul, int h32) {
    unsigned short zh, zm, zl;
    split3(-zmul, zh, zm, zl);
    if (h32 == (D / 8) % 2)
        qf[0][D / 16] = __builtin_bit_cast(bf16x8, make_uint4((unsigned)zh | ((unsigned)zm << 16), (unsigned)zl, 0u, 0u));
}

template <int D>
__device__ __forceinline__ v16f score_tile_q1(const unsigned short* kb, const bf16x8 (&qf)[3][Geo<D>::NKK], float zmul, int lane) {
    using G = Geo<D, 2, false>;
    v16f acc;
#pragma unroll
    for (int r = 0; r < 16; ++r) acc[r] = 0.0f;
    const unsigned short* kp = kb + (lane & 31) * G::KLD + 8 * (lane >> 5);
    constexpr int PL = KT * G::KLD;
#pragma unroll
    for (int kk = 0; kk < G::NKK; ++kk) {
        const bf16x8 kh = *reinterpret_cast<const bf16x8*>(kp + 16 * kk);
        const bf16x8 km = *reinterpret_cast<const bf16x8*>(kp + PL + 16 * kk);
        const bf16x8 kl = *reinterpret_cast<const bf16x8*>(kp + 2 * PL + 16 * kk);
        acc = __builtin_amdgcn_mfma_f32_32x32x16_bf16(kl, qf[0][kk], acc, 0, 0, 0);
        acc = __builtin_amdgcn_mfma_f32_32x32x16_bf16(km, qf[0][kk], acc, 0, 0, 0);
        acc = __builtin_amdgcn_mfma_f32_32x32x16_bf16(kh, qf[0][kk], acc, 0, 0, 0);
    }
    if constexpr (!G::FOLDZ) {
        const float* tv = reinterpret_cast<const float*>(kb + 3 * PL);
        const int h32 = lane >> 5;
#pragma unroll
        for (int g = 0; g < 4; ++g) {
            const float4 t4 = *reinterpret_cast<const float4*>(tv + 8 * g + 4 * h32);
            acc[4 * g + 0] = fmaf(-zmul, t4.x, acc[4 * g + 0]);
            acc[4 * g + 1] = fmaf(-zmul, t4.y, acc[4 * g + 1]);
            acc[4 * g + 2] = fmaf(-zmul, t4.z, acc[4 * g + 2]);
            acc[4 * g + 3] = fmaf(-zmul, t4.w, acc[4 * g + 3]);
        }
    }
    return acc;
}

__device__ __forceinline__ void attn_block_coords(int xcd_remap, int& bx, int& bh) {
    bx = blockIdx.x; bh = blockIdx.y;
    if (xcd_remap) {
        const int gx = gridDim.x, T = gridDim.x * gridDim.y;
        const int bid = blockIdx.x + gx * blockIdx.y;
        const int q = T >> 3, r = T & 7, xcd = bid & 7;
        const int logical = (xcd < r ? xcd * (q + 1) : r * (q + 1) + (xcd - r) * q) + (bid >> 3);
        bh = logical / gx;
        bx = logical - bh * gx;
    }
}

template <typename TIn> struct TypedLd {
    __device__ __forceinline__ void load8(const void* base, int64_t i, float (&x)[8]) const { ::load8<TIn>(reinterpret_cast<const TIn*>(base) + i, x); }
    __device__ __forceinline__ float load1(const void* base, int64_t i) const { return dgq_to_float(reinterpret_cast<const TIn*>(base)[i]); }
};
struct RtLd {
    int dtype;
    __device__ __forceinline__ void load8(const void* base, int64_t i, float (&x)[8]) const {
        if (dtype == DGQ_F16) ::load8<__half>(reinterpret_cast<const __half*>(base) + i, x);
        else if (dtype == DGQ_BF16) ::load8<__hip_bfloat16>(reinterpret_cast<const __hip_bfloat16*>(base) + i, x);
        else ::load8<float>(reinterpret_cast<const float*>(base) + i, x);
    }
    __device__ __forceinline__ float load1(const void* base, int64_t i) const { return load_any(base, dtype, i); }
};

template <int D, int QM, bool VINT, typename LD>
__device__ __forceinline__ void prep_k_tile(const LD& ld, const void* kp, int64_t kbase, int64_t HD, int S, int s0, const FqDesc& fk,
                                            const FqDesc& fqq, unsigned short* kimg, int tid) {
    using G = Geo<D, QM, VINT>;
    constexpr bool QI8 = QM == 1;
    if (QI8) {
        int8_t* k8 = reinterpret_cast<int8_t*>(kimg);
        float* ktab = reinterpret_cast<float*>(k8 + G::K8_BYTES);
        const int r = tid >> 3, part = tid & 7;
        const int sidx = s0 + r;
        const bool quant = sidx < S && sidx >= fk.skip;
        float dl = 0.0f, z = 0.0f, inv = 0.0f;
        if (quant) {
            const int idx = fk.mode == 0 ? 0 : sidx - fk.skip;
            dl = fk.delta[idx]; z = fk.zp[idx]; inv = dgq_rcp(dl);
        }
        const float off = 0.5f * (fk.qmax + 1.0f);
        float csum = 0.0f;
        for (int c8 = part; c8 < G::K8_LD / 8; c8 += 8) {
            unsigned w0 = 0, w1 = 0;
            if (quant && 8 * c8 < D) {
                float x[8];
                ld.load8(kp, kbase + sidx * HD + 8 * c8, x);
#pragma unroll
                for (int j = 0; j < 8; ++j) {
                    const float c = fq_code(x[j], dl, inv, z, fk.qmax, off);
                    csum += c;
                    const unsigned byte = ((unsigned)(int)c) & 0xFFu;
                    if (j < 4) w0 |= byte << (8 * j); else w1 |= byte << (8 * (j - 4));
                }
            }
            *reinterpret_cast<uint2*>(k8 + r * G::K8_LD + 8 * c8) = make_uint2(w0, w1);
        }
#pragma unroll
        for (int o = 4; o > 0; o >>= 1) csum += __shfl_xor(csum, o, 64);
        if (part == 0) {
            ktab[r] = dl;
            ktab[KT + r] = quant ? -(z - off) : 0.0f;
            ktab[2 * KT + r] = -csum;
        }
    }
    constexpr int KC = G::KLD / 8;
    if (QM == 2) {
        const int r = tid >> 3, part = tid & 7;
        const int sidx = s0 + r;
        const float offq = 0.5f * (fqq.qmax + 1.0f);
        float corr = 0.0f;
        constexpr int KIT = (KC + 7) / 8;
        float x[KIT][8];
#pragma unroll
        for (int it = 0; it < KIT; ++it)
            if (sidx < S && 8 * (part + 8 * it) < D) ld.load8(kp, kbase + sidx * HD + 8 * (part + 8 * it), x[it]);
#pragma unroll
        for (int it = 0; it < KIT; ++it) {
            const int c8 = part + 8 * it;
            if (c8 >= KC) continue;
            unsigned wh[4] = {0, 0, 0, 0}, wm[4] = {0, 0, 0, 0}, wl[4] = {0, 0, 0, 0};
            if (sidx < S && 8 * c8 < D) {
                fq_apply8(fk, x[it], sidx, 8 * c8);
#pragma unroll
                for (int j = 0; j < 8; ++j) {
                    if (fqq.mode == 2) {
                        x[it][j] *= fqq.delta[8 * c8 + j];
                        corr += (fqq.zp[8 * c8 + j] - offq) * x[it][j];
                    } else {
                        corr += x[it][j];
                    }
                }
#pragma unroll
                for (int j = 0; j < 4; ++j) {
                    unsigned short h0, m0, l0, h1, m1, l1;
                    split3(x[it][2 * j], h0, m0, l0);
                    split3(x[it][2 * j + 1], h1, m1, l1);
                    wh[j] = (unsigned)h0 | ((unsigned)h1 << 16);
                    wm[j] = (unsigned)m0 | ((unsigned)m1 << 16);
                    wl[j] = (unsigned)l0 | ((unsigned)l1 << 16);
                }
            }
            unsigned short* dst = kimg + r * G::KLD + 8 * c8;
            *reinterpret_cast<uint4*>(dst) = make_uint4(wh[0], wh[1], wh[2], wh[3]);
            *reinterpret_cast<uint4*>(dst + KT * G::KLD) = make_uint4(wm[0], wm[1], wm[2], wm[3]);
            *reinterpret_cast<uint4*>(dst + 2 * KT * G::KLD) = make_uint4(wl[0], wl[1], wl[2], wl[3]);
        }
#pragma unroll
        for (int o = 4; o > 0; o >>= 1) corr += __shfl_xor(corr, o, 64);
        if (part == 0) reinterpret_cast<float*>(kimg + 3 * KT * G::KLD)[r] = corr;
        if (G::FOLDZ && part == (D / 8) % 8) {
            unsigned short th, tm, tl;
            split3(corr, th, tm, tl);
            unsigned short* dst = kimg + r * G::KLD + D;
            *reinterpret_cast<uint2*>(dst) = make_uint2((unsigned)th | ((unsigned)th << 16), (unsigned)th);
            *reinterpret_cast<uint2*>(dst + KT * G::KLD) = make_uint2((unsigned)tm | ((unsigned)tm << 16), (unsigned)tm);
            *reinterpret_cast<uint2*>(dst + 2 * KT * G::KLD) = make_uint2((unsigned)tl | ((unsigned)tl << 16), (unsigned)tl);
        }
    }
    for (int i = tid; QM == 0 && i < KT * KC; i += 256) {
        const int r = i / KC, c8 = i - r * KC;
        const int sidx = s0 + r;
        unsigned wh[4], wm[4], wl[4];
        const bool live = sidx < S && 8 * c8 < D;
        float x[8];
        if (live) {
            ld.load8(kp, kbase + sidx * HD + 8 * c8, x);
            fq_apply8(fk, x, sidx, 8 * c8);
        }
#pragma unroll
        for (int j = 0; j < 4; ++j) {
            unsigned short h0 = 0, m0 = 0, l0 = 0, h1 = 0, m1 = 0, l1 = 0;
            if (live) {
                split3(x[2 * j], h0, m0, l0);
                split3(x[2 * j + 1], h1, m1, l1);
            }
            wh[j] = (unsigned)h0 | ((unsigned)h1 << 16);
            wm[j] = (unsigned)m0 | ((unsigned)m1 << 16);
            wl[j] = (unsigned)l0 | ((unsigned)l1 << 16);
        }
        unsigned short* dst = kimg + r * G::KLD + 8 * c8;
        *reinterpret_cast<uint4*>(dst) = make_uint4(wh[0], wh[1], wh[2], wh[3]);
        *reinterpret_cast<uint4*>(dst + KT * G::KLD) = make_uint4(wm[0], wm[1], wm[2], wm[3]);
        *reinterpret_cast<uint4*>(dst + 2 * KT * G::KLD) = make_uint4(wl[0], wl[1], wl[2], wl[3]);
    }
}

template <int D, int QM, bool VINT, typename LD>
__device__ __forceinline__ void prep_v_tile(const LD& ld, const void* vp, int64_t vbase, int64_t HD, int S, int s0, const FqDesc& fv,
                                            unsigned short* vimg, int tid) {
    using G = Geo<D, QM, VINT>;
    constexpr int VC = G::VLD / 8;
    constexpr int VIT = (G::DV * VC + 255) / 256;
    {
        float xv[VIT][8];
#pragma unroll
        for (int it = 0; it < VIT; ++it) {
            const int i = tid + 256 * it;
            const int c8 = i / G::DV, d = i - c8 * G::DV;
#pragma unroll
            for (int s8 = 0; s8 < 8; ++s8) {
                const int sidx = s0 + 16 * (c8 >> 1) + 8 * (s8 >> 2) + 4 * (c8 & 1) + (s8 & 3);
                xv[it][s8] = (c8 < 4 && sidx < S && d < D) ? ld.load1(vp, vbase + sidx * HD + d) : 0.0f;
            }
        }
#pragma unroll
        for (int it = 0; it < VIT; ++it) {
            const int i = tid + 256 * it;
            if (i >= G::DV * VC) continue;
            const int c8 = i / G::DV, d = i - c8 * G::DV;
            unsigned wh[4], wm[4], wl[4];
#pragma unroll
            for (int j = 0; j < 4; ++j) {
                unsigned short hh[2] = {0, 0}, mm[2] = {0, 0}, ll[2] = {0, 0};
#pragma unroll
                for (int e = 0; e < 2; ++e) {
                    const int slot8 = 2 * j + e;
                    const int sidx = s0 + 16 * (c8 >> 1) + 8 * (slot8 >> 2) + 4 * (c8 & 1) + (slot8 & 3);
                    if (G::VONES && c8 < 4 && d == D) hh[e] = 0x3F80;
                    if (c8 < 4 && sidx < S && d < D) {
                        const float x1 = xv[it][slot8];
                        if (VINT) {
                            const int idx = fv.mode == 0 ? 0 : d;
                            const float dl = fv.delta[idx];
                            hh[e] = bf16_bits(fq_code(x1, dl, dgq_rcp(dl), fv.zp[idx], fv.qmax, 0.5f * (fv.qmax + 1.0f)));
                        } else {
                            split3(fq_apply(fv, x1, sidx, d), hh[e], mm[e], ll[e]);
                        }
                    }
                }
                wh[j] = (unsigned)hh[0] | ((unsigned)hh[1] << 16);
                wm[j] = (unsigned)mm[0] | ((unsigned)mm[1] << 16);
                wl[j] = (unsigned)ll[0] | ((unsigned)ll[1] << 16);
            }
            unsigned short* dst = vimg + d * G::VLD + 8 * c8;
            *reinterpret_cast<uint4*>(dst) = make_uint4(wh[0], wh[1], wh[2], wh[3]);
            if (!VINT) {
                *reinterpret_cast<uint4*>(dst + G::DV * G::VLD) = make_uint4(wm[0], wm[1], wm[2], wm[3]);
                *reinterpret_cast<uint4*>(dst + 2 * G::DV * G::VLD) = make_uint4(wl[0], wl[1], wl[2], wl[3]);
            }
        }
    }
}

int dgq_attention_one_launch(const AttnParams& p, int D, int qm, bool vint, unsigned* sync, hipStream_t st);
```

### dgq_amd/ops.py

```python
import ctypes
import os
import threading
from typing import Optional

import torch
import torch.nn.functional as F

from . import _lib
from .plan import ActLayout, natural_kperm, round_up, KTILE, act_offset, mark_clears, flush_coefficients

_c = ctypes


def _lib_call(name, *args):
    _lib.check(getattr(_lib.load(), name)(*args), name)


def quantize_weight(w: torch.Tensor, delta: torch.Tensor, zp: torch.Tensor, alpha: Optional[torch.Tensor], bits: int):
    _lib.require_gpu()
    N = w.shape[0]
    w2 = w.detach().reshape(N, -1).contiguous().float()
    K = w2.shape[1]
    d = delta.detach().reshape(-1).contiguous().float()
    z = zp.detach().reshape(-1).contiguous().float()
    assert d.numel() == N and z.numel() == N, "weight quantizer must be per output channel"
    a = alpha.detach().reshape(N, -1).contiguous().float() if alpha is not None else None
    codes = torch.empty((N, K), dtype=torch.uint8, device=w.device)
    _lib_call("dgq_quantize_weight", _lib.ptr(w2), _lib.ptr(d), _lib.ptr(z), _lib.ptr(a), N, K, bits,
              _lib.ptr(codes), _lib.stream())
    return codes


class _AdaRoundSoft(torch.autograd.Function):

    @staticmethod
    def forward(ctx, w2, d, z, alpha2, bits):
        N, K = w2.shape
        out = torch.empty_like(w2)
        _lib_call("dgq_adaround_soft_fwd", _lib.ptr(w2), _lib.ptr(d), _lib.ptr(z), _lib.ptr(alpha2), N, K, bits,
                  _lib.ptr(out), _lib.stream())
        ctx.save_for_backward(w2, d, z, alpha2)
        ctx.bits = bits
        return out

    @staticmethod
    def backward(ctx, gout):
        w2, d, z, alpha2 = ctx.saved_tensors
        N, K = w2.shape
        g = gout.contiguous().float()
        galpha = torch.empty_like(alpha2)
        _lib_call("dgq_adaround_soft_bwd", _lib.ptr(g), _lib.ptr(w2), _lib.ptr(d), _lib.ptr(z), _lib.ptr(alpha2), N, K,
                  ctx.bits, _lib.ptr(galpha), _lib.stream())
        return None, None, None, galpha, None


def adaround_soft(w: torch.Tensor, delta: torch.Tensor, zp: torch.Tensor, alpha: torch.Tensor, bits: int):
    _lib.require_gpu()
    N = w.shape[0]
    w2 = w.detach().reshape(N, -1).contiguous().float()
    d = delta.detach().reshape(-1).contiguous().float()
    z = torch.as_tensor(zp).detach().reshape(-1).float().to(w.device)
    z = (z.expand(N) if z.numel() == 1 else z).contiguous()
    assert d.numel() == N and z.numel() == N, "weight quantizer must be per output channel"
    a2 = alpha.reshape(N, -1)
    if a2.dtype != torch.float32 or not a2.is_contiguous():
        a2 = a2.float().contiguous()
    return _AdaRoundSoft.apply(w2, d, z, a2, bits).view(w.shape)


class _AdaRoundReg(torch.autograd.Function):

    @staticmethod
    def forward(ctx, alpha, b):
        a = alpha.contiguous()
        n = a.numel()
        part = torch.empty((_lib.load().dgq_adaround_reg_blocks(n),), dtype=torch.float32, device=a.device)
        _lib_call("dgq_adaround_reg_fwd", _lib.ptr(a), n, _c.c_float(b), _lib.ptr(part), _lib.stream())
        ctx.save_for_backward(a)
        ctx.b = b
        return part.sum()

    @staticmethod
    def backward(ctx, g):
        (a,) = ctx.saved_tensors
        gs = g.reshape(1).float().contiguous()
        galpha = torch.empty_like(a)
        _lib_call("dgq_adaround_reg_bwd", _lib.ptr(a), a.numel(), _c.c_float(ctx.b), _lib.ptr(gs), _lib.ptr(galpha),
                  _lib.stream())
        return galpha.view_as(a), None


def adaround_reg(alpha: torch.Tensor, b: float):
    _lib.require_gpu()
    assert alpha.dtype == torch.float32
    return _AdaRoundReg.apply(alpha, float(b))


W4_LAYOUT = 1


W4_FRAG_LAYOUT = 2
GEMM_PANEL = True


def pack_weight(codes: torch.Tensor, kperm: Optional[torch.Tensor], Kp: int, bits: int, layout: int = W4_LAYOUT):
    N, K = codes.shape
    kp = kperm.to(codes.device, torch.int32).contiguous() if kperm is not None else None
    if bits == 4:
        rows = (N + 31) // 32 * 32 if layout == W4_FRAG_LAYOUT else N
        out = torch.empty((rows, Kp // 2), dtype=torch.uint8, device=codes.device)
        _lib_call("dgq_pack_w4", _lib.ptr(codes), N, K, _lib.ptr(kp), Kp, layout, _lib.ptr(out), _lib.stream())
    elif bits == 8:
        out = torch.empty((N, Kp), dtype=torch.int8, device=codes.device)
        _lib_call("dgq_pack_w8", _lib.ptr(codes), N, K, _lib.ptr(kp), Kp, _lib.ptr(out), _lib.stream())
    else:
        raise NotImplementedError("weight bits %d: the HIP path implements W4 and W8" % bits)
    return out


def unpack_w4(packed: torch.Tensor, Kp: int, layout: int = W4_LAYOUT):
    N = packed.shape[0]
    out = torch.empty((N, Kp), dtype=torch.uint8, device=packed.device)
    _lib_call("dgq_unpack_w4", _lib.ptr(packed), N, Kp, layout, _lib.ptr(out), _lib.stream())
    return out


class PackedWeight:

    def __init__(self, w, delta, zp, alpha, bias, bits, C, taps):
        self.bits, self.C, self.taps = bits, C, taps
        self.N = w.shape[0]
        self.K = C * taps
        dev = w.device
        self.codes = quantize_weight(w, delta, zp, alpha, bits)
        woff = 0.0 if bits == 4 else 128.0
        self.alpha = delta.detach().reshape(-1).float().contiguous().to(dev)
        self.zp_true = zp.detach().reshape(-1).float().contiguous().to(dev)
        self.zw = (self.zp_true - woff).contiguous()
        self.bias = (bias.detach().float().contiguous().to(dev) if bias is not None
                     else torch.zeros(self.N, device=dev))
        self._natural = None
        self._natural_frag = None
        self._vn = None

    def natural_frag(self):
        if self._natural_frag is None and self.bits == 4 and GEMM_PANEL:
            perm = natural_kperm(self.C, self.taps)
            self._natural_frag = pack_weight(self.codes, perm, perm.numel(), 4, W4_FRAG_LAYOUT)
        return self._natural_frag

    def natural(self):
        if self._natural is None:
            perm = natural_kperm(self.C, self.taps)
            self._natural = (pack_weight(self.codes, perm, perm.numel(), self.bits), perm.numel())
        return self._natural

    def centered(self):
        return self.codes.double() - self.zp_true.double()[:, None]

    def vn(self):
        if self._vn is None:
            self._vn = self.centered().sum(dim=1).float().contiguous()
        return self._vn


class ActBinding:

    def koff(self, W, ldc):
        if self.ksrc is None:
            return None
        key = (W, ldc)
        if key not in self._koff:
            e = self.ksrc
            off = (((e >> 24) & 0x7F) * W + ((e >> 16) & 0xFF)) * ldc + (e & 0xFFFF)
            self._koff[key] = torch.where(e >= 0, off, torch.full_like(off, -1)).to(torch.int32).contiguous()
        return self._koff[key]

    def klds(self, kw, C):
        if self.ksrc is None:
            return None
        key = ("lds", kw, C)
        if key not in self._koff:
            e = self.ksrc
            idx = (((e >> 24) & 0x7F) * kw + ((e >> 16) & 0xFF)) * C + (e & 0xFFFF)
            self._koff[key] = torch.where(e >= 0, idx, torch.full_like(idx, -1)).to(torch.int32).contiguous()
        return self._koff[key]

    def kdst(self, kw, C, taps):
        if self.ksrc is None:
            return None
        key = ("dst", kw, C, taps)
        if key not in self._koff:
            e = self.ksrc
            valid = e >= 0
            idx = ((((e >> 24) & 0x7F) * kw + ((e >> 16) & 0xFF)) * C + (e & 0xFFFF))[valid].long()
            out = torch.full((taps * C,), -1, dtype=torch.int32, device=e.device)
            out[idx] = torch.nonzero(valid).flatten().to(torch.int32)
            assert int((out < 0).sum()) == 0, "per-K table does not cover every (tap, channel)"
            self._koff[key] = out.contiguous()
        return self._koff[key]

    def kpat(self, kh, kw, C, stride):
        key = ("pat", kh, kw, C, stride)
        if key not in self._koff:
            pw_ = _c.c_int(0)
            tile = _lib.load().dgq_quant_act_conv_tile(C, kh, kw, stride, self.Kp, _c.byref(pw_))
            if tile == 0:
                self._koff[key] = None
            elif self.ksrc is not None:
                e = self.ksrc
                idx = (((e >> 24) & 0x7F) * pw_.value + ((e >> 16) & 0xFF)) * C + (e & 0xFFFF)
                self._koff[key] = torch.where(e >= 0, idx, torch.full_like(idx, -1)).to(torch.int32).contiguous()
            else:
                kp = torch.arange(self.Kp, device=self.pw.codes.device)
                tap, c = kp // C, kp % C
                idx = ((tap // kw) * pw_.value + (tap % kw)) * C + c
                self._koff[key] = torch.where(kp < kh * kw * C, idx, torch.full_like(idx, -1)).to(torch.int32).contiguous()
        return self._koff[key]

    def kpat_for(self, kh, kw, C, pw):
        key = ("patw", kh, kw, C, pw)
        if key not in self._koff:
            if self.ksrc is not None:
                e = self.ksrc
                idx = (((e >> 24) & 0x7F) * pw + ((e >> 16) & 0xFF)) * C + (e & 0xFFFF)
                self._koff[key] = torch.where(e >= 0, idx, torch.full_like(idx, -1)).to(torch.int32).contiguous()
            else:
                kp = torch.arange(self.Kp, device=self.pw.codes.device)
                tap, c = kp // C, kp % C
                idx = ((tap // kw) * pw + (tap % kw)) * C + c
                self._koff[key] = torch.where(kp < kh * kw * C, idx, torch.full_like(idx, -1)).to(torch.int32).contiguous()
        return self._koff[key]

    def input_binding(self, C):
        hit = self._koff.get(("input", C))
        if hit is None:
            import copy
            hit = copy.copy(self)
            hit.Kp = round_up(C, KTILE)
            hit._koff = {}
            self._koff[("input", C)] = hit
        return hit

    def conv_zero_code(self):
        return self._zc

    def conv_fill(self):
        return self._fill

    def __init__(self, layout: ActLayout, pw: PackedWeight, abits: int):
        dev = pw.codes.device
        self.mode, self.abits, self.offset = layout.mode, abits, act_offset(abits)
        self.pw = pw
        if layout.mode == "perK":
            self.Kp = layout.Kp
            self.ksrc = layout.ksrc.to(dev)
            self._koff = {}
            self.cdelta = layout.cdelta.to(dev)
            self.czp = layout.czp.to(dev)
            cfl = mark_clears(layout.cflush, abits, pw.bits)
            self.cflush = cfl.to(dev)
            self.ccoef = flush_coefficients(layout.cdelta, cfl).to(dev)
            self.wpacked = pack_weight(pw.codes, layout.kperm, layout.Kp, pw.bits)
            self.wfrag = pack_weight(pw.codes, layout.kperm, layout.Kp, 4, W4_FRAG_LAYOUT) if (pw.bits == 4 and GEMM_PANEL) else None
            U = (pw.centered() @ layout.kcoef.to(dev)).float()
            self.gamma = (pw.bias + pw.alpha * U).contiguous()
            self.n_groups = layout.n_groups
        else:
            self.wpacked, self.Kp = pw.natural()
            self.wfrag = pw.natural_frag()
            self.ksrc = None
            self._koff = {}
            self.mdelta = layout.mdelta.to(dev).contiguous()
            self.mzp = layout.mzp.to(dev).contiguous()
            self.L = layout.L
            self.gamma = pw.bias
            self.vn = pw.vn()
            if layout.mode == "scalar":
                z = float(layout.mzp.reshape(-1)[0])
                if 0.0 <= round(z) <= 2.0 ** abits - 1.0:
                    self._zc = float(round(z) - self.offset)
                    self._fill = torch.tensor([int(self._zc)] * 16 + [0] * 16, dtype=torch.int8, device=dev)
                else:
                    self._zc, self._fill = None, None


def act_ksplits(M, Kp):
    ks = max(1, min(16, 8192 // max(M, 1), Kp // 512))
    return _lib.load().dgq_quant_act_parts(Kp, ks)


FLOAT_DTYPES = (torch.float32, torch.float16, torch.bfloat16)
def as_f32(t: torch.Tensor) -> torch.Tensor:
    if t.dtype == torch.float32:
        return t.detach()
    key = (t._version, t.data_ptr(), t.dtype)
    hit = t.__dict__.get("_dgq_f32")
    if hit is None or hit[0] != key:
        hit = (key, t.detach().float().contiguous())
        t.__dict__["_dgq_f32"] = hit
    return hit[1]


def groupnorm_scale_shift(x_cl: torch.Tensor, B, HW, C, groups, eps, gamma, beta):
    dev = x_cl.device
    slices = max(1, min(32, (2048 + B * groups - 1) // (B * groups), HW // 64))
    scale = torch.empty((B, C), dtype=torch.float32, device=dev)
    shift = torch.empty((B, C), dtype=torch.float32, device=dev)
    part = torch.empty((B * groups * slices * 3,), dtype=torch.float32, device=dev)
    _lib_call("dgq_groupnorm_scale_shift", _lib.ptr(x_cl), _lib.DTYPE_CODE[x_cl.dtype], B, HW, C, groups,
              _c.c_float(eps), _lib.ptr(as_f32(gamma)), _lib.ptr(as_f32(beta)), _lib.ptr(scale), _lib.ptr(shift),
              _lib.ptr(part), slices, _lib.stream())
    return scale, shift


GN_FROM_GEMM = True
GN_FROM_SPLITK = True


CONV_IMPLICIT = True


class OutputRedirect:

    def __init__(self, out=None, out2=None):
        self.out, self.out2, self.taken = out, out2, False


_REDIRECT_TLS = threading.local()


def set_redirect(rd):
    _REDIRECT_TLS.rd = rd


def pending_redirect():
    return getattr(_REDIRECT_TLS, "rd", None)


CAT_INPLACE = os.environ.get("DGQ_CAT_INPLACE", "1") != "0"


def take_redirect(M, N, dtype):
    rd = pending_redirect()
    if rd is None or rd.taken:
        return None, None
    for v in (rd.out, rd.out2):
        if v is not None and (tuple(v.shape) != (M, N) or v.dtype != dtype or v.stride(1) != 1):
            return None, None
    rd.taken = True
    return rd.out, rd.out2


def cat_channels(a: torch.Tensor, b: torch.Tensor) -> torch.Tensor:
    y = torch.cat([a, b], dim=1)
    ga, gb = _gn_of(a), _gn_of(b)
    if ga is not None and gb is not None and len(ga["parts"]) == 1 and len(gb["parts"]) == 1 and ga["B"] == gb["B"] and ga["HW"] == gb["HW"]:
        y._dgq_gn = dict(parts=ga["parts"] + gb["parts"], B=ga["B"], HW=ga["HW"], C=ga["C"] + gb["C"], ver=y._version)
    return y


def _gn_of(x: torch.Tensor):
    gn = getattr(x, "_dgq_gn", None) if GN_FROM_GEMM else None
    return gn if (gn is not None and gn.get("ver") == x._version) else None


def groupnorm_from_partials(gn, groups, eps, gamma, beta):
    parts = gn["parts"]
    B, HW, C = gn["B"], gn["HW"], gn["C"]
    dev = parts[0][0].device
    scale = torch.empty((B, C), dtype=torch.float32, device=dev)
    shift = torch.empty((B, C), dtype=torch.float32, device=dev)
    p2, c2 = (parts[1][0], parts[1][1]) if len(parts) > 1 else (None, 0)
    _lib_call("dgq_groupnorm_from_partials", _lib.ptr(parts[0][0]), parts[0][1], _lib.ptr(p2), c2, B, HW, groups, _c.c_float(eps),
              _lib.ptr(as_f32(gamma)), _lib.ptr(as_f32(beta)), _lib.ptr(scale), _lib.ptr(shift), _lib.stream())
    return scale, shift


def quant_act(x_cl: torch.Tensor, B, H, W, C, kh, kw, stride, pad, ab: ActBinding, pre=None, ln=None, ups=False):
    Ho = (H + 2 * pad - kh) // stride + 1
    Wo = (W + 2 * pad - kw) // stride + 1
    M = B * Ho * Wo
    per_m = 0 if ab.mode == "perK" else 1
    ldc = 2 * C if (pre and pre[2] == 2) else C
    a = _lib.QuantActArgs()
    a.x, a.x_dtype, a.B, a.H, a.W, a.C, a.kh, a.kw, a.stride, a.pad = x_cl.data_ptr(), _lib.DTYPE_CODE[x_cl.dtype], B, H, W, C, kh, kw, stride, pad
    a.ksrc, a.koff, a.klds = _dp(ab.ksrc), _dp(ab.koff(W, ldc)), _dp(ab.klds(kw, C))
    a.kdst = _dp(ab.kdst(kw, C, kh * kw)) if ab.ksrc is not None else None
    a.kpat = _dp(ab.kpat(kh, kw, C, stride)) if (kh * kw > 1 and C % 4 == 0) else None
    a.Kp, a.per_m = ab.Kp, per_m
    a.delta, a.zp = (ab.cdelta.data_ptr(), ab.czp.data_ptr()) if not per_m else (ab.mdelta.data_ptr(), ab.mzp.data_ptr())
    a.L, a.bits = (1 if not per_m else ab.L), ab.abits
    a.pre_scale = _dp(pre[0]) if pre and pre[0] is not None else None
    a.pre_shift = _dp(pre[1]) if pre and pre[1] is not None else None
    a.pre_act = pre[2] if pre else 0
    lnp = (as_f32(ln[0]), as_f32(ln[1]), float(ln[2])) if ln else None
    a.ln_gamma, a.ln_beta, a.ln_eps = (lnp[0].data_ptr(), lnp[1].data_ptr(), lnp[2]) if lnp else (None, None, 0.0)
    a.ups = 1 if ups else 0
    parts = 1
    a.ksplits = 1
    a.codes = a.rowsum = 1
    if (a.kdst is None and a.kpat is None) or _lib.load().dgq_quant_act_variant(_c.byref(a)) not in (3, 4, 5):
        if ups:
            return None
        parts = act_ksplits(M, ab.Kp)
        a.ksplits = parts
    codes = torch.empty((M, ab.Kp), dtype=torch.int8, device=x_cl.device)
    rowsum = torch.empty((parts, M), dtype=torch.float32, device=x_cl.device)
    a.codes, a.rowsum = codes.data_ptr(), rowsum.data_ptr()

    def issue():
        _lib_call("dgq_quant_act_batch", 1, _c.byref(a), _lib.stream())
    issue()
    if QUANT_LAUNCH_HOOK is not None:
        QUANT_LAUNCH_HOOK(issue, B * H * W * ldc * x_cl.element_size() >> (2 if ups else 0), M * ab.Kp + 4 * parts * M)
    return codes, rowsum, M


def _dp(t):
    return t.data_ptr() if t is not None else None


_WORKSPACE = {}
WORKSPACE_BYTES = 128 << 20
_STREAM_SLABS_MAX = 4


def workspace(device):
    cur = torch.cuda.current_stream(device).cuda_stream
    is_main = cur == torch.cuda.default_stream(device).cuda_stream or torch.cuda.is_current_stream_capturing()
    branch = "main" if is_main else ("stream", cur)
    key = (str(device), branch)
    if key not in _WORKSPACE:
        if torch.cuda.is_current_stream_capturing():
            raise RuntimeError("dgq_amd: the split-K workspace must exist before graph capture (run the model once eagerly)")
        if isinstance(branch, tuple):
            old = [k for k in _WORKSPACE if k[0] == str(device) and isinstance(k[1], tuple)]
            while len(old) >= _STREAM_SLABS_MAX:
                _WORKSPACE.pop(old.pop(0))
        _WORKSPACE[key] = torch.empty(WORKSPACE_BYTES, dtype=torch.uint8, device=device)
    elif isinstance(branch, tuple):
        _WORKSPACE[key] = _WORKSPACE.pop(key)
    return _WORKSPACE[key]


def make_extra(residual=None, fq=None, res_div=1, geglu=False, gn_partial=None, conv=None, y2=None):
    if residual is None and fq is None and not geglu and gn_partial is None and conv is None and y2 is None:
        return None
    ex = _lib.GemmExtra()
    ex.res_div = 1
    if y2 is not None:
        assert y2.dim() == 2 and y2.stride(1) == 1
        ex.y2, ex.ldy2 = y2.data_ptr(), y2.stride(0)
        ex._y2_keep = y2
    ex.conv = None
    ex.flush_coef = None
    if conv is not None:
        ex.conv = _c.cast(_c.pointer(conv[0]), _c.c_void_p)
        ex._conv_keep = conv
    ex.geglu = 1 if geglu else 0
    ex.gn_partial = gn_partial.data_ptr() if gn_partial is not None else None
    keep = []
    if residual is not None:
        assert residual.dtype in _lib.DTYPE_CODE and residual.stride(-1) == 1
        ex.residual, ex.ldr, ex.res_div = residual.data_ptr(), residual.stride(0), res_div
        ex.res_dtype = _lib.DTYPE_CODE[residual.dtype]
        keep.append(residual)
    if gn_partial is not None:
        keep.append(gn_partial)
    if fq is not None:
        mode, delta, zp, T, D, skip, bits = fq
        ex.fq_mode, ex.fq_delta, ex.fq_zp = mode, delta.data_ptr(), zp.data_ptr()
        ex.fq_T, ex.fq_D, ex.fq_skip, ex.fq_qmax = T, D, skip, float(2 ** bits - 1)
        keep += [delta, zp]
    else:
        ex.fq_T = ex.fq_D = 1
    ex._keep = keep
    return ex


QUANT_LAUNCH_HOOK = None
ATTN_LAUNCH_HOOK = None
GEMM_LAUNCH_HOOK = None


def with_layer_tables(extra, ab: "ActBinding", M):
    need_coef = ab.mode == "perK" and M >= 2048 and ab.pw.N >= 128
    wfrag = getattr(ab, "wfrag", None)
    if not need_coef and wfrag is None:
        return extra
    if extra is None:
        extra = _lib.GemmExtra()
        extra.res_div, extra.fq_T, extra.fq_D, extra._keep = 1, 1, 1, []
    if need_coef:
        extra.flush_coef = ab.ccoef.data_ptr()
    if wfrag is not None:
        extra.wfrag = wfrag.data_ptr()
    return extra


GEMM_FUSE = True
CONV_FUSE = os.environ.get("DGQ_CONV_FUSE", "1") != "0"


def _act_operand_ok(x2):
    return x2 is None or (x2.data_ptr() % 16 == 0 and (x2.stride(0) * x2.element_size()) % 8 == 0 and x2.stride(-1) == 1)


def act_fuses(ab: "ActBinding", M, K, dtype, n_problems=1, x2=None, N=None, Kp=None):
    if not (GEMM_FUSE and GEMM_PANEL) or getattr(ab, "wfrag", None) is None or ab.pw.taps != 1 or K % 4 != 0 or dtype not in _lib.DTYPE_CODE:
        return False
    if not _act_operand_ok(x2):
        return False
    dt = _lib.DTYPE_CODE[dtype]
    return bool(_lib.load().dgq_gemm_act_fuses(M, ab.pw.N if N is None else N, K, ab.Kp if Kp is None else Kp, ab.pw.bits,
                                               0 if ab.mode == "perK" else 1, n_problems, dt, dt))


def _multi_fuses(bindings, M, Kin, dtype, x2):
    groups = {}
    for i, ab in enumerate(bindings):
        if ab.pw.K != Kin:
            return False
        groups.setdefault(0 if ab.mode == "perK" else 1, []).append(ab)
    for abs_ in groups.values():
        for j0 in range(0, len(abs_), 8):
            chunk = abs_[j0:j0 + 8]
            kp = max(ab.Kp for ab in chunk)
            if not all(act_fuses(ab, M, Kin, dtype, len(chunk), x2, N=chunk[0].pw.N, Kp=kp) for ab in chunk):
                return False
    return True


def conv_act_fuses(ab: "ActBinding", B, H, W, C, kh, kw, stride, pad, dtype, x_store=None):
    if not (GEMM_FUSE and CONV_FUSE) or getattr(ab, "wfrag", None) is None or ab.mode == "scalar" or dtype not in _lib.DTYPE_CODE:
        return False
    if x_store is not None and not (x_store.is_contiguous() and x_store.data_ptr() % 16 == 0 and (C * x_store.element_size()) % 8 == 0):
        return False
    dt = _lib.DTYPE_CODE[dtype]
    return bool(_lib.load().dgq_gemm_conv_act_fuses(B, H, W, C, kh, kw, stride, pad, ab.pw.N, ab.Kp, ab.pw.bits,
                                                    0 if ab.mode == "perK" else 1, dt, dt))


def make_act(x2: torch.Tensor, ab: "ActBinding", pre=None, ln=None, rows_per_image=1):
    K = ab.pw.K
    a = _lib.GemmAct()
    a.x, a.x_dtype, a.ldx, a.K = x2.data_ptr(), _lib.DTYPE_CODE[x2.dtype], x2.stride(0), K
    keep = [x2]
    if ab.mode == "perK":
        kd = ab.kdst(1, K, 1)
        a.kdst, a.czp = kd.data_ptr(), ab.czp.data_ptr()
        keep.append(kd)
    a.bits = ab.abits
    a.rows_per_image, a.pre_act = rows_per_image, 0
    if pre is not None:
        if pre[0] is not None:
            a.pre_scale, a.pre_shift = pre[0].data_ptr(), pre[1].data_ptr()
            keep += [pre[0], pre[1]]
        a.pre_act = pre[2]
    if ln is not None:
        g, b = as_f32(ln[0]), as_f32(ln[1])
        a.ln_gamma, a.ln_beta, a.ln_eps = g.data_ptr(), b.data_ptr(), float(ln[2])
        keep += [g, b]
    a._keep = keep
    return a


def gemm_act(x2, M, ab: "ActBinding", out_dtype, extra=None, pre=None, ln=None, rows_per_image=1, out=None):
    act = make_act(x2, ab, pre, ln, rows_per_image)
    extra = with_layer_tables(extra, ab, M)
    extra.act = _c.cast(_c.pointer(act), _c.c_void_p)
    extra._act_keep = act
    dummy = ab.wfrag
    return gemm_wxa8(dummy, dummy, M, ab, out_dtype, out=out, extra=extra, _fused_bytes=x2.element_size() * M * ab.pw.K)


def gemm_wxa8(codes, rowsum, M, ab: ActBinding, out_dtype, out: Optional[torch.Tensor] = None, extra=None, _fused_bytes=0):
    pw = ab.pw
    ws = workspace(codes.device)
    extra = with_layer_tables(extra, ab, M)
    if out is None:
        out = torch.empty((M, pw.N // 2 if (extra is not None and extra.geglu) else pw.N), dtype=out_dtype, device=codes.device)
    per_m = 0 if ab.mode == "perK" else 1
    parts = rowsum.shape[0] if (rowsum.dim() == 2 and not _fused_bytes) else 1
    def issue():
        _lib_call("dgq_gemm_wxa8", _lib.ptr(codes), _lib.ptr(rowsum), parts, M, ab.Kp, _lib.ptr(ab.wpacked), pw.bits, pw.N,
                  per_m,
                  _lib.ptr(ab.cdelta) if not per_m else None, _lib.ptr(ab.cflush) if not per_m else None,
                  _lib.ptr(ab.mdelta) if per_m else None, _lib.ptr(ab.mzp) if per_m else None,
                  ab.L if per_m else 1, _c.c_float(ab.offset),
                  _lib.ptr(pw.alpha), _lib.ptr(pw.zw), _lib.ptr(ab.gamma), _lib.ptr(ab.vn) if per_m else None,
                  _lib.ptr(out), _lib.DTYPE_CODE[out.dtype], out.stride(0), _lib.ptr(ws), ws.numel(),
                  _c.byref(extra) if extra is not None else None, _lib.stream())
    issue()
    if GEMM_LAUNCH_HOOK is not None:
        GEMM_LAUNCH_HOOK(issue, [(M, ab, out.element_size(), _fused_bytes)])
    return out


def quant_linear(x: torch.Tensor, ab: ActBinding, pre_act=0, residual=None, fq=None, ln=None, geglu=False):
    Kin = x.shape[-1]
    K = Kin // 2 if pre_act == 2 else Kin
    x2 = x.reshape(-1, Kin)
    if not x2.is_contiguous():
        x2 = x2.contiguous()
    rows = x2.shape[0]
    pre = (None, None, pre_act) if pre_act else None
    res2 = None
    if residual is not None:
        res2 = residual.reshape(-1, ab.pw.N)
        if not res2.is_contiguous():
            res2 = res2.contiguous()
    if pre_act != 2 and act_fuses(ab, rows, K, x.dtype, x2=x2):
        y = gemm_act(x2, rows, ab, x.dtype, extra=make_extra(res2, fq, geglu=geglu), pre=pre, ln=ln)
        return y.view(*x.shape[:-1], y.shape[-1])
    codes, rowsum, M = quant_act(x2, rows, 1, 1, K, 1, 1, 1, 0, ab, pre, ln)
    y = gemm_wxa8(codes, rowsum, M, ab, x.dtype, extra=make_extra(res2, fq, geglu=geglu))
    return y.view(*x.shape[:-1], y.shape[-1])


def _quant_linear_multi_fused(x, x2, M, bindings, ln):
    dev = x2.device
    outs = [torch.empty((M, ab.pw.N), dtype=x.dtype, device=dev) for ab in bindings]
    groups = {}
    for i, ab in enumerate(bindings):
        groups.setdefault(0 if ab.mode == "perK" else 1, []).append(i)
    for per_m, idxs in groups.items():
        for j0 in range(0, len(idxs), 8):
            chunk = idxs[j0:j0 + 8]
            arr = (_lib.GemmArgs * len(chunk))()
            extras = []
            for g, i in zip(arr, chunk):
                ab, pw = bindings[i], bindings[i].pw
                act = make_act(x2, ab, None, ln)
                ex = with_layer_tables(None, ab, 0)
                ex.act = _c.cast(_c.pointer(act), _c.c_void_p)
                extras.append((ex, act))
                g.codes, g.rowsum, g.rowsum_parts, g.M, g.Kp = ab.wfrag.data_ptr(), ab.wfrag.data_ptr(), 1, M, ab.Kp
                g.wpacked, g.w_bits, g.N, g.per_m = ab.wpacked.data_ptr(), pw.bits, pw.N, per_m
                g.cdelta, g.cflush = (ab.cdelta.data_ptr(), ab.cflush.data_ptr()) if not per_m else (None, None)
                g.mdelta, g.mzp = (ab.mdelta.data_ptr(), ab.mzp.data_ptr()) if per_m else (None, None)
                g.L, g.offset = (ab.L if per_m else 1), ab.offset
                g.alpha, g.zw, g.gamma, g.vn = pw.alpha.data_ptr(), pw.zw.data_ptr(), ab.gamma.data_ptr(), (ab.vn.data_ptr() if per_m else None)
                g.y, g.y_dtype, g.ldy = outs[i].data_ptr(), _lib.DTYPE_CODE[outs[i].dtype], outs[i].stride(0)
                g.extra = _c.cast(_c.pointer(ex), _c.c_void_p)
            n_chunk = len(chunk)

            def issue(arr=arr, n_chunk=n_chunk, _keep=extras):
                _lib_call("dgq_gemm_wxa8_batch", n_chunk, _c.cast(arr, _c.c_void_p), _lib.stream())
            issue()
            if GEMM_LAUNCH_HOOK is not None:
                GEMM_LAUNCH_HOOK(issue, [(M, bindings[i], outs[i].element_size(), (M * bindings[i].pw.K * x2.element_size()) if j == 0 else 0)
                                         for j, i in enumerate(chunk)])
    return [o.view(*x.shape[:-1], o.shape[-1]) for o in outs]


def quant_linear_multi(x: torch.Tensor, bindings, ln=None):
    Kin = x.shape[-1]
    x2 = x.reshape(-1, Kin)
    if not x2.is_contiguous():
        x2 = x2.contiguous()
    M = x2.shape[0]
    dev = x2.device
    lib = _lib.load()
    if _multi_fuses(bindings, M, Kin, x.dtype, x2):
        return _quant_linear_multi_fused(x, x2, M, bindings, ln)
    lnp = (as_f32(ln[0]), as_f32(ln[1]), float(ln[2])) if ln else None
    qa, keep = [], []
    for ab in bindings:
        assert ab.pw.K == Kin and ab.pw.taps == 1
        per_m = 0 if ab.mode == "perK" else 1
        a = _lib.QuantActArgs()
        a.x, a.x_dtype, a.B, a.H, a.W, a.C, a.kh, a.kw, a.stride, a.pad = x2.data_ptr(), _lib.DTYPE_CODE[x2.dtype], M, 1, 1, Kin, 1, 1, 1, 0
        a.ksrc, a.koff, a.klds = _dp(ab.ksrc), _dp(ab.koff(1, Kin)), _dp(ab.klds(1, Kin))
        a.kdst = _dp(ab.kdst(1, Kin, 1)) if ab.ksrc is not None else None
        a.Kp, a.per_m = ab.Kp, per_m
        a.delta, a.zp = (ab.cdelta.data_ptr(), ab.czp.data_ptr()) if not per_m else (ab.mdelta.data_ptr(), ab.mzp.data_ptr())
        a.L, a.bits = (1 if not per_m else ab.L), ab.abits
        a.pre_scale = a.pre_shift = None
        a.pre_act = 0
        a.ln_gamma, a.ln_beta, a.ln_eps = (lnp[0].data_ptr(), lnp[1].data_ptr(), lnp[2]) if lnp else (None, None, 0.0)
        a.codes = a.rowsum = 1
        parts, a.ksplits = 1, 1
        if a.kdst is None or lib.dgq_quant_act_variant(_c.byref(a)) not in (3, 4):
            parts = act_ksplits(M, ab.Kp)
            a.ksplits = parts
        codes = torch.empty((M, ab.Kp), dtype=torch.int8, device=dev)
        rowsum = torch.empty((parts, M), dtype=torch.float32, device=dev)
        a.codes, a.rowsum = codes.data_ptr(), rowsum.data_ptr()
        variant = lib.dgq_quant_act_variant(_c.byref(a))
        qa.append((variant, per_m, a, codes, rowsum, parts))
    groups = {}
    for i, (variant, per_m, a, *_rest) in enumerate(qa):
        groups.setdefault((variant, per_m), []).append(i)
    for idxs in groups.values():
        for j0 in range(0, len(idxs), 8):
            chunk = idxs[j0:j0 + 8]
            arr = (_lib.QuantActArgs * len(chunk))(*[qa[i][2] for i in chunk])

            def issue_q(arr=arr, n_chunk=len(chunk)):
                _lib_call("dgq_quant_act_batch", n_chunk, _c.cast(arr, _c.c_void_p), _lib.stream())
            issue_q()
            if QUANT_LAUNCH_HOOK is not None:
                QUANT_LAUNCH_HOOK(issue_q, M * Kin * x2.element_size(), sum(M * bindings[i].Kp + 4 * qa[i][5] * M for i in chunk))
    outs = [torch.empty((M, ab.pw.N), dtype=x.dtype, device=dev) for ab in bindings]
    ggroups = {}
    for i, ab in enumerate(bindings):
        ggroups.setdefault((qa[i][1], ab.pw.bits), []).append(i)
    for (per_m, _bits), idxs in ggroups.items():
        for j0 in range(0, len(idxs), 8):
            chunk = idxs[j0:j0 + 8]
            arr = (_lib.GemmArgs * len(chunk))()
            extras = []
            for g, i in zip(arr, chunk):
                ab, pw = bindings[i], bindings[i].pw
                _v, _pm, _a, codes, rowsum, parts = qa[i]
                g.codes, g.rowsum, g.rowsum_parts, g.M, g.Kp = codes.data_ptr(), rowsum.data_ptr(), parts, M, ab.Kp
                g.wpacked, g.w_bits, g.N, g.per_m = ab.wpacked.data_ptr(), pw.bits, pw.N, per_m
                g.cdelta, g.cflush = (ab.cdelta.data_ptr(), ab.cflush.data_ptr()) if not per_m else (None, None)
                g.mdelta, g.mzp = (ab.mdelta.data_ptr(), ab.mzp.data_ptr()) if per_m else (None, None)
                g.L, g.offset = (ab.L if per_m else 1), ab.offset
                g.alpha, g.zw, g.gamma, g.vn = pw.alpha.data_ptr(), pw.zw.data_ptr(), ab.gamma.data_ptr(), (ab.vn.data_ptr() if per_m else None)
                ex = with_layer_tables(None, ab, 0)
                extras.append(ex)
                g.y, g.y_dtype, g.ldy = outs[i].data_ptr(), _lib.DTYPE_CODE[outs[i].dtype], outs[i].stride(0)
                g.extra = _c.cast(_c.pointer(ex), _c.c_void_p) if ex is not None else None
            n_chunk = len(chunk)

            def issue(arr=arr, n_chunk=n_chunk, _keep=extras):
                _lib_call("dgq_gemm_wxa8_batch", n_chunk, _c.cast(arr, _c.c_void_p), _lib.stream())
            issue()
            if GEMM_LAUNCH_HOOK is not None:
                GEMM_LAUNCH_HOOK(issue, [(M, bindings[i], outs[i].element_size(), 0) for i in chunk])
    keep.append(qa)
    return [o.view(*x.shape[:-1], o.shape[-1]) for o in outs]


def quant_conv2d(x: torch.Tensor, ab: ActBinding, kh, kw, stride, pad, norm=None, residual=None, bias_rows=None, gn_out=True, upsample=False,
                 out=None, out2=None):
    if upsample and (norm is not None or ab.mode == "scalar" or kh * kw == 1):
        x, upsample = F.interpolate(x, scale_factor=2.0, mode="nearest"), False
    B, C, H, W = x.shape
    if upsample:
        H, W = 2 * H, 2 * W
    xc = x.contiguous(memory_format=torch.channels_last)
    x_store = xc.permute(0, 2, 3, 1)
    pre = None
    if norm is not None:
        groups, eps, gamma, beta, act = norm
        gn = _gn_of(x)
        if gn is not None and gn["B"] == B and gn["HW"] == H * W and gn["C"] == C and C % groups == 0:
            sc, sh = groupnorm_from_partials(gn, groups, eps, gamma, beta)
        else:
            sc, sh = groupnorm_scale_shift(x_store, B, H * W, C, groups, eps, gamma, beta)
        pre = (sc, sh, act)
    Ho = (H + 2 * pad - kh) // stride + 1
    Wo = (W + 2 * pad - kw) // stride + 1
    M = B * Ho * Wo
    res2, res_div = None, 1
    if residual is not None:
        res2 = residual.contiguous(memory_format=torch.channels_last).permute(0, 2, 3, 1).reshape(M, ab.pw.N)
    elif bias_rows is not None:
        res2, res_div = bias_rows.contiguous(), M // B
    N = ab.pw.N
    if kh == 1 and kw == 1 and stride == 1 and pad == 0 and act_fuses(ab, M, C, x.dtype, x2=x_store.reshape(M, C)):
        part = torch.empty((M // 16, N, 2), dtype=torch.float32, device=x.device) if (GN_FROM_GEMM and gn_out and (Ho * Wo) % 16 == 0 and N % 4 == 0) else None
        y = gemm_act(x_store.reshape(M, C), M, ab, x.dtype, extra=make_extra(res2, res_div=res_div, gn_partial=part, y2=out2), pre=pre, rows_per_image=H * W,
                     out=out)
        out = y.view(B, Ho, Wo, N).permute(0, 3, 1, 2)
        if part is not None:
            out._dgq_gn = dict(parts=[(part, N)], B=B, HW=Ho * Wo, C=N, ver=out._version)
        return out
    if kh * kw > 1 and not upsample and conv_act_fuses(ab, B, H, W, C, kh, kw, stride, pad, x.dtype, x_store):
        part = torch.empty((M // 16, N, 2), dtype=torch.float32, device=x.device) if (GN_FROM_GEMM and gn_out and (Ho * Wo) % 16 == 0 and N % 4 == 0) else None
        act = _lib.GemmAct()
        kp_ = ab.kpat_for(kh, kw, C, 8 + kw - 1)
        act.x, act.x_dtype, act.ldx, act.K = x_store.data_ptr(), _lib.DTYPE_CODE[x_store.dtype], C, C
        act.kpat, act.bits, act.rows_per_image, act.pre_act = kp_.data_ptr(), ab.abits, H * W, 0
        act.B, act.H, act.W, act.kh, act.kw, act.stride, act.pad = B, H, W, kh, kw, stride, pad
        act._keep = [x_store, kp_]
        if ab.mode == "perK":
            act.czp = ab.czp.data_ptr()
        if pre is not None:
            if pre[0] is not None:
                act.pre_scale, act.pre_shift = pre[0].data_ptr(), pre[1].data_ptr()
                act._keep += [pre[0], pre[1]]
            act.pre_act = pre[2]
        extra = with_layer_tables(make_extra(res2, res_div=res_div, gn_partial=part, y2=out2), ab, M)
        extra.act = _c.cast(_c.pointer(act), _c.c_void_p)
        extra._act_keep = act
        y = gemm_wxa8(ab.wfrag, ab.wfrag, M, ab, x.dtype, out=out, extra=extra, _fused_bytes=x.element_size() * B * H * W * C)
        out = y.view(B, Ho, Wo, N).permute(0, 3, 1, 2)
        if part is not None:
            out._dgq_gn = dict(parts=[(part, N)], B=B, HW=Ho * Wo, C=N, ver=out._version)
        return out
    implicit = CONV_IMPLICIT and ab.mode == "scalar" and kh * kw > 1 and C % 16 == 0 and ab.pw.bits == 4 and ab.conv_zero_code() is not None
    conv_desc = None
    if implicit:
        abi = ab.input_binding(C)
        codes, pixsum, _ = quant_act(x_store, B, H, W, C, 1, 1, 1, 0, abi, pre)
        rowsum = torch.empty((1, M), dtype=torch.float32, device=x.device)
        cv = _lib.GemmConv()
        cv.codes_in, cv.pixsum, cv.fill = codes.data_ptr(), pixsum.data_ptr(), ab.conv_fill().data_ptr()
        cv.B, cv.H, cv.W, cv.C, cv.ldc, cv.kh, cv.kw, cv.stride, cv.pad, cv.Ho, cv.Wo = B, H, W, C, abi.Kp, kh, kw, stride, pad, Ho, Wo
        cv.zero_code, cv.pixsum_parts = ab.conv_zero_code(), pixsum.shape[0]
        conv_desc = (cv, pixsum)
    else:
        qa = quant_act(x_store, B, H, W, C, kh, kw, stride, pad, ab, pre, ups=upsample)
        if qa is None:
            return quant_conv2d(F.interpolate(x, scale_factor=2.0, mode="nearest"), ab, kh, kw, stride, pad, norm=norm, residual=residual,
                                bias_rows=bias_rows, gn_out=gn_out, out=out, out2=out2)
        codes, rowsum, M = qa
    N = ab.pw.N
    part = None
    if (GN_FROM_GEMM and gn_out and (Ho * Wo) % 16 == 0 and N % 4 == 0 and
            (GN_FROM_SPLITK or _lib.load().dgq_gemm_plan_splits(M, N, ab.Kp, ab.pw.bits, 0 if ab.mode == "perK" else 1, WORKSPACE_BYTES) == 1)):
        part = torch.empty((M // 16, N, 2), dtype=torch.float32, device=x.device)
    y = gemm_wxa8(codes, rowsum, M, ab, x.dtype, out=out, extra=make_extra(res2, res_div=res_div, gn_partial=part, conv=conv_desc, y2=out2))
    out = y.view(B, Ho, Wo, N).permute(0, 3, 1, 2)
    if part is not None:
        out._dgq_gn = dict(parts=[(part, N)], B=B, HW=Ho * Wo, C=N, ver=out._version)
    return out


def conv2d_f32w(x: torch.Tensor, w_nat: torch.Tensor, bias, kh, kw, stride, pad, norm=None, out2=None, gn_out=False):
    N = w_nat.shape[0]
    is_conv = x.dim() == 4 and w_nat.shape[1] == kh * kw * x.shape[1]
    if x.dim() == 4 and not is_conv:
        assert kh == kw == 1 and w_nat.shape[1] == x.shape[-1], "dgq conv2d_f32w: weight [N][%d] does not match input %s" % (w_nat.shape[1], tuple(x.shape))
    if is_conv:
        B, C, H, W = x.shape
        xs = x.contiguous(memory_format=torch.channels_last)
        sc = sh = None
        act = 0
        if norm is not None:
            groups, eps, gamma, beta, act = norm
            gn = _gn_of(x)
            if gn is not None and gn["B"] == B and gn["HW"] == H * W and gn["C"] == C and C % groups == 0:
                sc, sh = groupnorm_from_partials(gn, groups, eps, gamma, beta)
            else:
                sc, sh = groupnorm_scale_shift(xs.permute(0, 2, 3, 1), B, H * W, C, groups, eps, gamma, beta)
        Ho = (H + 2 * pad - kh) // stride + 1
        Wo = (W + 2 * pad - kw) // stride + 1
        y = torch.empty((B * Ho * Wo, N), dtype=x.dtype, device=x.device)
        part = None
        if gn_out and GN_FROM_GEMM and (Ho * Wo) % 16 == 0 and N % 4 == 0 and N > 8:
            part = torch.empty((B * Ho * Wo // 16, N, 2), dtype=torch.float32, device=x.device)
        _lib_call("dgq_conv2d_f32w", _lib.ptr(xs), _lib.DTYPE_CODE[x.dtype], B, H, W, C, kh, kw, stride, pad,
                  _lib.ptr(w_nat), _lib.ptr(bias), N, _lib.ptr(y), _lib.DTYPE_CODE[y.dtype], N,
                  _lib.ptr(sc), _lib.ptr(sh), int(act), _lib.ptr(out2), out2.stride(0) if out2 is not None else 0, _lib.ptr(part), _lib.stream())
        out = y.view(B, Ho, Wo, N).permute(0, 3, 1, 2)
        if part is not None:
            out._dgq_gn = dict(parts=[(part, N)], B=B, HW=Ho * Wo, C=N, ver=out._version)
        return out
    K = x.shape[-1]
    assert w_nat.shape[1] == K and kh == kw == 1, "dgq conv2d_f32w: weight [N][%d] does not match input %s" % (w_nat.shape[1], tuple(x.shape))
    x2 = x.reshape(-1, K)
    if not x2.is_contiguous():
        x2 = x2.contiguous()
    y = torch.empty((x2.shape[0], N), dtype=x.dtype, device=x.device)
    assert norm is None
    _lib_call("dgq_conv2d_f32w", _lib.ptr(x2), _lib.DTYPE_CODE[x.dtype], x2.shape[0], 1, 1, K, 1, 1, 1, 0,
              _lib.ptr(w_nat), _lib.ptr(bias), N, _lib.ptr(y), _lib.DTYPE_CODE[y.dtype], N, None, None, 0, None, 0, None, _lib.stream())
    return y.view(*x.shape[:-1], N)


def conv2d_wq(x: torch.Tensor, pw: PackedWeight, kh, kw, stride, pad, upsample=False, geglu_rows=False):
    w_img, Kp = pw.natural()
    N = pw.N
    is_conv = x.dim() == 4 and pw.K == kh * kw * x.shape[1]
    if is_conv:
        B, C, H, W = x.shape
        if upsample:
            H, W = 2 * H, 2 * W
        xs = x.contiguous(memory_format=torch.channels_last)
        Ho = (H + 2 * pad - kh) // stride + 1
        Wo = (W + 2 * pad - kw) // stride + 1
        y = torch.empty((B * Ho * Wo, N), dtype=x.dtype, device=x.device)
        _lib_call("dgq_conv2d_wq", _lib.ptr(xs), _lib.DTYPE_CODE[x.dtype], B, H, W, C, kh, kw, stride, pad, int(upsample),
                  _lib.ptr(w_img), pw.bits, Kp, _lib.ptr(pw.alpha), _lib.ptr(pw.zp_true), _lib.ptr(pw.bias), N, int(geglu_rows),
                  _lib.ptr(y), _lib.DTYPE_CODE[y.dtype], N, _lib.stream())
        return y.view(B, Ho, Wo, N).permute(0, 3, 1, 2)
    K = x.shape[-1]
    assert pw.K == K and kh == kw == 1 and not upsample, "dgq conv2d_wq: weight [N][%d] does not match input %s" % (pw.K, tuple(x.shape))
    x2 = x.reshape(-1, K)
    if not x2.is_contiguous():
        x2 = x2.contiguous()
    y = torch.empty((x2.shape[0], N), dtype=x.dtype, device=x.device)
    _lib_call("dgq_conv2d_wq", _lib.ptr(x2), _lib.DTYPE_CODE[x.dtype], x2.shape[0], 1, 1, K, 1, 1, 1, 0, 0,
              _lib.ptr(w_img), pw.bits, Kp, _lib.ptr(pw.alpha), _lib.ptr(pw.zp_true), _lib.ptr(pw.bias), N, int(geglu_rows),
              _lib.ptr(y), _lib.DTYPE_CODE[y.dtype], N, _lib.stream())
    return y.view(*x.shape[:-1], N)


def fakequant_rows(x2d: torch.Tensor, T, D, mode, delta, zp, skip, bits, out=None):
    assert x2d.is_contiguous()
    rows, C = x2d.shape
    out = x2d if out is None else out
    _lib_call("dgq_fakequant_rows", _lib.ptr(x2d), _lib.ptr(out), _lib.DTYPE_CODE[x2d.dtype], rows, C, T, D, mode,
              _lib.ptr(delta), _lib.ptr(zp), skip, bits, _lib.stream())
    return out


def timestep_embedding(timesteps: torch.Tensor, dim: int, out_dtype=torch.float32):
    assert timesteps.dim() == 1 and timesteps.dtype in (torch.int64, torch.float32) and dim % 2 == 0
    rows = timesteps.shape[0]
    out = torch.empty((rows, dim), dtype=out_dtype, device=timesteps.device)
    _lib_call("dgq_timestep_embedding", _lib.ptr(timesteps), 1 if timesteps.dtype == torch.float32 else 0, int(timesteps.stride(0)), rows, dim,
              _lib.ptr(out), _lib.DTYPE_CODE[out_dtype], _lib.stream())
    return out


def _dense_layout(t):
    if t.is_contiguous():
        return 0
    if t.dim() == 4 and t.is_contiguous(memory_format=torch.channels_last):
        return 1
    return None


def cfg_ddim_step(eps_uncond, eps_cond, sample, guidance, s1, inv_s2, s3, s4):
    lay = _dense_layout(eps_uncond)
    if (lay is None or not sample.is_contiguous() or sample.dim() < 2 or eps_uncond.shape != sample.shape
            or (eps_cond is not None and (eps_cond.shape != sample.shape or _dense_layout(eps_cond) != lay))):
        return None
    for t in (eps_uncond, eps_cond):
        assert t is None or t.dtype == sample.dtype
    C = sample.shape[1]
    HW = sample.numel() // (sample.shape[0] * C)
    out = torch.empty_like(sample)
    _lib_call("dgq_cfg_ddim_step", _lib.ptr(eps_uncond), _lib.ptr(eps_cond), _lib.ptr(sample), _lib.ptr(out), _lib.DTYPE_CODE[sample.dtype], sample.numel(), C, HW, lay,
              _c.c_float(guidance), _c.c_float(s1), _c.c_float(inv_s2), _c.c_float(s3), _c.c_float(s4), _lib.stream())
    return out


def max_f32(p: torch.Tensor, skip_cols=0):
    assert p.is_contiguous() and p.dtype == torch.float32
    S = p.shape[-1]
    rows = p.numel() // S
    out = torch.zeros((1,), dtype=torch.float32, device=p.device)
    _lib_call("dgq_max_f32", _lib.ptr(p), rows, S, skip_cols, _lib.ptr(out), _lib.stream())
    return out


def logquant_f32(p: torch.Tensor, delta: torch.Tensor, bits, skip_cols=0, out=None):
    assert p.is_contiguous() and p.dtype == torch.float32
    S = p.shape[-1]
    rows = p.numel() // S
    out = p if out is None else out
    _lib_call("dgq_logquant_f32", _lib.ptr(p), _lib.ptr(out), rows, S, skip_cols, _lib.ptr(delta), bits, _lib.stream())
    return out


SMALLM_MAX_M, SMALLM_MAX_K, SMALLM_MAX_PROBLEMS = 16, 2048, 24


def linear_smallm_batch(x2d: torch.Tensor, bindings, pre_act=0):
    assert x2d.dim() == 2 and x2d.stride(1) == 1 and x2d.dtype in _lib.DTYPE_CODE
    M, K = x2d.shape
    outs = []
    for i0 in range(0, len(bindings), SMALLM_MAX_PROBLEMS):
        chunk = bindings[i0:i0 + SMALLM_MAX_PROBLEMS]
        probs = (_lib.SmallMProblem * len(chunk))()
        keep = []
        for j, ab in enumerate(chunk):
            pw = ab.pw
            assert ab.mode != "perK" and ab.L == 1 and pw.K == K and pw.taps == 1
            y = torch.empty((M, pw.N), dtype=x2d.dtype, device=x2d.device)
            q = probs[j]
            q.wpacked, q.alpha, q.zw = ab.wpacked.data_ptr(), pw.alpha.data_ptr(), pw.zw.data_ptr()
            q.gamma, q.vn = ab.gamma.data_ptr(), ab.vn.data_ptr()
            q.mdelta, q.mzp = ab.mdelta.data_ptr(), ab.mzp.data_ptr()
            q.y, q.ldy, q.N, q.Kp, q.w_bits, q.a_bits = y.data_ptr(), y.stride(0), pw.N, ab.Kp, pw.bits, ab.abits
            keep.append(y)
        _lib_call("dgq_linear_smallm_batch", _lib.ptr(x2d), _lib.DTYPE_CODE[x2d.dtype], M, K, x2d.stride(0), pre_act,
                  len(chunk), _c.cast(probs, _c.c_void_p), _lib.DTYPE_CODE[x2d.dtype], _lib.stream())
        outs += keep
    return outs


def minmax_rows_cols(x2d: torch.Tensor, rows=True, cols=True):
    assert x2d.dim() == 2 and x2d.stride(1) == 1 and x2d.dtype in _lib.DTYPE_CODE
    R, C = x2d.shape
    dev = x2d.device
    rmin = rmax = cmin = cmax = part = None
    slices = max(1, min(256, R // 64))
    if rows:
        rmin = torch.empty((R,), dtype=torch.float32, device=dev)
        rmax = torch.empty((R,), dtype=torch.float32, device=dev)
    if cols:
        cmin = torch.empty((C,), dtype=torch.float32, device=dev)
        cmax = torch.empty((C,), dtype=torch.float32, device=dev)
        part = torch.empty((2 * slices * C,), dtype=torch.float32, device=dev)
    _lib_call("dgq_minmax_rows_cols", _lib.ptr(x2d), _lib.DTYPE_CODE[x2d.dtype], R, C, x2d.stride(0),
              _lib.ptr(rmin), _lib.ptr(rmax), _lib.ptr(cmin), _lib.ptr(cmax), _lib.ptr(part), slices, _lib.stream())
    return rmin, rmax, cmin, cmax


ATTN_HEAD_DIMS = (8, 16, 40, 64, 80, 160)
_ATTN_WS = {}


def _attn_workspace(device, nbytes):
    cap = torch.cuda.is_current_stream_capturing()
    key = (str(device), torch.cuda.current_stream(device).cuda_stream if not cap else "capture")
    buf = _ATTN_WS.get(key)
    if buf is None or buf.numel() < nbytes:
        buf = torch.empty((max(nbytes, 1 << 20),), dtype=torch.uint8, device=device)
        if not cap:
            _ATTN_WS[key] = buf
    return buf


def attention_fuses_fakequant(D, mode):
    return bool(_lib.load().dgq_attention_fuses_fakequant(D, mode))


def attention(q, k, v, H, D, scale, mode, skip, delta, bits, fq=None):
    assert q.dtype in _lib.DTYPE_CODE and k.dtype == q.dtype and v.dtype == q.dtype
    assert q.is_contiguous() and k.is_contiguous() and v.is_contiguous()
    B, T, _ = q.shape
    S = k.shape[1]
    nbytes = _lib.load().dgq_attention_workspace_bytes(B, H, T, S, D)
    ws = _attn_workspace(q.device, nbytes)
    desc = None
    if fq is not None and any(f is not None for f in fq):
        desc = (_lib.AttnFq * 3)()
        for i, f in enumerate(fq):
            if f is None:
                desc[i].mode = -1
                continue
            fmode, fd, fz, fskip, fbits = f
            ntok = (T if i == 0 else S) - fskip
            need = 1 if fmode == 0 else (ntok if fmode == 1 else D)
            assert fd.numel() == need and fz.numel() == need and fd.dtype == torch.float32 and fd.is_contiguous(), \
                "q/k/v quantizer table has %d entries, kernel addresses %d" % (fd.numel(), need)
            desc[i].mode, desc[i].skip, desc[i].bits = fmode, fskip, fbits
            desc[i].delta, desc[i].zero_point = _lib.ptr(fd), _lib.ptr(fz)
    o = torch.empty_like(q)

    def issue():
        _lib_call("dgq_attention", _lib.ptr(q), _lib.ptr(k), _lib.ptr(v), _lib.ptr(o), _lib.DTYPE_CODE[q.dtype], B, H, T, S, D,
                  _c.c_float(scale), mode, skip, _lib.ptr(delta), bits,
                  _c.cast(desc, _c.c_void_p) if desc is not None else None, _lib.ptr(ws), nbytes, _lib.stream())
    issue()
    if ATTN_LAUNCH_HOOK is not None:
        ATTN_LAUNCH_HOOK(issue, 4.0 * T * S * D * B * H, (2 * B * T + 2 * B * S) * H * D * q.element_size())
    return o


attention_f32 = attention


def attention_sync_timeouts():
    n = _lib.load().dgq_attention_sync_timeouts()
    if n < 0:
        raise RuntimeError("dgq_attention_sync_timeouts failed")
    return n
```

### include/dgq_hip.h

```cpp
#ifndef DGQ_HIP_H
#define DGQ_HIP_H
#include <stddef.h>
#include <stdint.h>

#ifdef __cplusplus
extern "C" {
#endif

#define DGQ_OK 0
#define DGQ_EINVAL (-1)
#define DGQ_EUNSUPPORTED (-2)
#define DGQ_ELAUNCH (-3)

#define DGQ_F32 0
#define DGQ_F16 1
#define DGQ_BF16 2

#define DGQ_KCHUNK 32
#define DGQ_KTILE 128

#define DGQ_ABI_VERSION 123
int dgq_version(void);
const char* dgq_last_error(void);

int dgq_quantize_weight(const float* w, const float* delta, const float* zp, const float* alpha,
                        int N, int K, int bits, uint8_t* codes, void* stream);

int dgq_pack_w4(const uint8_t* codes, int N, int K, const int32_t* kperm, int Kp, int layout, uint8_t* packed, void* stream);
int dgq_unpack_w4(const uint8_t* packed, int N, int Kp, int layout, uint8_t* out, void* stream);
int dgq_pack_w8(const uint8_t* codes, int N, int K, const int32_t* kperm, int Kp, int8_t* packed, void* stream);

int dgq_quant_act(const void* x, int x_dtype, int B, int H, int W, int C,
                  int kh, int kw, int stride, int pad,
                  const int32_t* ksrc, const int32_t* koff, const int32_t* klds, int Kp,
                  int per_m, const float* delta, const float* zp, int L,
                  int bits, int8_t* codes, float* rowsum, int ksplits,
                  const float* pre_scale, const float* pre_shift, int pre_act,
                  const float* ln_gamma, const float* ln_beta, float ln_eps, void* stream);
int dgq_quant_act_parts(int Kp, int ksplits);
typedef struct dgq_quant_act_args {
    const void* x; int x_dtype; int B, H, W, C, kh, kw, stride, pad;
    const int32_t* ksrc; const int32_t* koff; const int32_t* klds;
    const int32_t* kdst;
    int Kp;
    int per_m; const float* delta; const float* zp; int L; int bits;
    int8_t* codes; float* rowsum; int ksplits;
    const float* pre_scale; const float* pre_shift; int pre_act;
    const float* ln_gamma; const float* ln_beta; float ln_eps;
    const int32_t* kpat;
    int ups;
} dgq_quant_act_args_t;
int dgq_quant_act_batch(int n, const dgq_quant_act_args_t* args, void* stream);
int dgq_quant_act_variant(const dgq_quant_act_args_t* args);
int dgq_quant_act_conv_tile(int C, int kh, int kw, int stride, int Kp, int* patch_w);

int dgq_groupnorm_scale_shift(const void* x, int x_dtype, int B, int HW, int C, int G, float eps,
                              const float* gamma, const float* beta, float* scale, float* shift,
                              float* partial_ws, int slices, void* stream);
int dgq_groupnorm_from_partials(const float* partial, int C1, const float* partial2, int C2, int B, int HW, int G, float eps,
                                const float* gamma, const float* beta, float* scale, float* shift, void* stream);

int dgq_timestep_embedding(const void* t, int t_is_float, int64_t t_stride, int rows, int dim, void* out, int out_dtype, void* stream);
int dgq_cfg_ddim_step(const void* eps_uncond, const void* eps_cond, const void* sample, void* out, int dtype, int64_t n, int C, int HW,
                      int eps_channels_last, float guidance, float s1, float inv_s2, float s3, float s4, void* stream);

int dgq_conv2d_f32w(const void* x, int x_dtype, int B, int H, int W, int C, int kh, int kw, int stride, int pad,
                    const float* w, const float* bias, int N, void* y, int y_dtype, int ldy,
                    const float* pre_scale, const float* pre_shift, int pre_act, void* y2, int ldy2, float* gn_partial, void* stream);

int dgq_conv2d_wq(const void* x, int x_dtype, int B, int H, int W, int C, int kh, int kw, int stride, int pad, int upsample,
                  const uint8_t* w_packed, int w_bits, int Kp, const float* delta, const float* zp, const float* bias, int N,
                  int geglu_rows, void* y, int y_dtype, int ldy, void* stream);

typedef struct dgq_gemm_conv {
    const int8_t* codes_in;
    const float* pixsum;
    const int8_t* fill;
    int B, H, W, C, ldc, kh, kw, stride, pad, Ho, Wo;
    float zero_code;
    int pixsum_parts;
} dgq_gemm_conv_t;

typedef struct dgq_gemm_act {
    const void* x; int x_dtype; int ldx; int K;
    const int32_t* kdst; const float* czp; int bits;
    const float* pre_scale; const float* pre_shift; int rows_per_image; int pre_act;
    const float* ln_gamma; const float* ln_beta; float ln_eps;
    const int32_t* kpat; int B, H, W, kh, kw, stride, pad;
} dgq_gemm_act_t;

typedef struct dgq_gemm_extra {
    const void* residual;
    int ldr;
    int res_div;
    int res_dtype;
    int fq_mode;
    const float* fq_delta;
    const float* fq_zp;
    int fq_T, fq_D, fq_skip;
    float fq_qmax;
    int geglu;
    float* gn_partial;
    const dgq_gemm_conv_t* conv;
    const float* flush_coef;
    const void* wfrag;
    const dgq_gemm_act_t* act;
    void* y2;
    int ldy2;
} dgq_gemm_extra_t;

int dgq_gemm_wxa8(const int8_t* codes, const float* rowsum, int rowsum_parts, int M, int Kp,
                  const void* wpacked, int w_bits, int N,
                  int per_m, const float* cdelta, const uint8_t* cflush,
                  const float* mdelta, const float* mzp, int L, float offset,
                  const float* alpha, const float* zw, const float* gamma, const float* vn,
                  void* y, int y_dtype, int ldy, void* workspace, size_t workspace_bytes,
                  const dgq_gemm_extra_t* extra, void* stream);
int dgq_gemm_act_fuses(int M, int N, int K, int Kp, int w_bits, int per_m, int n_problems, int x_dtype, int y_dtype);
int dgq_gemm_conv_act_fuses(int B, int H, int W, int C, int kh, int kw, int stride, int pad, int N, int Kp, int w_bits, int per_m,
                            int x_dtype, int y_dtype);
typedef struct dgq_gemm_args {
    const int8_t* codes; const float* rowsum; int rowsum_parts; int M, Kp;
    const void* wpacked; int w_bits; int N;
    int per_m; const float* cdelta; const uint8_t* cflush; const float* mdelta; const float* mzp; int L; float offset;
    const float* alpha; const float* zw; const float* gamma; const float* vn;
    void* y; int y_dtype; int ldy;
    const dgq_gemm_extra_t* extra;
} dgq_gemm_args_t;
int dgq_gemm_wxa8_batch(int n, const dgq_gemm_args_t* args, void* stream);
size_t dgq_gemm_workspace_bytes(int M, int N, int Kp);
int dgq_gemm_plan_splits(int M, int N, int Kp, int w_bits, int per_m, size_t workspace_bytes);

int dgq_fakequant_rows(const void* x, void* y, int dtype, int rows, int C, int T, int D,
                       int mode, const float* delta, const float* zp, int skip, int bits, void* stream);

int dgq_max_f32(const float* p, int64_t rows, int S, int skip_cols, float* out, void* stream);
int dgq_logquant_f32(const float* p, float* y, int64_t rows, int S, int skip_cols, const float* delta,
                     int bits, void* stream);

typedef struct dgq_attn_fq {
    int mode;
    int skip;
    int bits;
    const float* delta;
    const float* zero_point;
} dgq_attn_fq_t;
int dgq_attention_f32(const float* q, const float* k, const float* v, float* o, int B, int H, int T, int S, int D,
                      float scale, int mode, int skip, const float* delta_in, int bits, const dgq_attn_fq_t* fq,
                      void* workspace, size_t workspace_bytes, void* stream);
int dgq_attention(const void* q, const void* k, const void* v, void* o, int dtype, int B, int H, int T, int S, int D,
                  float scale, int mode, int skip, const float* delta_in, int bits, const dgq_attn_fq_t* fq,
                  void* workspace, size_t workspace_bytes, void* stream);
int dgq_attention_fuses_fakequant(int D, int mode);
size_t dgq_attention_workspace_bytes(int B, int H, int T, int S, int D);
int dgq_attention_sync_timeouts(void);

typedef struct dgq_smallm_problem {
    const void* wpacked;
    const float* alpha;
    const float* zw;
    const float* gamma;
    const float* vn;
    const float* mdelta;
    const float* mzp;
    void* y;
    int ldy, N, Kp, w_bits, a_bits;
} dgq_smallm_problem_t;
int dgq_linear_smallm_batch(const void* x, int x_dtype, int M, int K, int64_t ldx, int pre_act, int n_problems,
                            const dgq_smallm_problem_t* probs, int y_dtype, void* stream);

int dgq_minmax_rows_cols(const void* x, int dtype, int rows, int C, int64_t ldx,
                         float* rowmin, float* rowmax, float* colmin, float* colmax,
                         float* partial_ws, int slices, void* stream);

int dgq_adaround_soft_fwd(const float* w, const float* delta, const float* zp, const float* alpha, int N, int K, int bits,
                          float* out, void* stream);
int dgq_adaround_soft_bwd(const float* gout, const float* w, const float* delta, const float* zp, const float* alpha, int N,
                          int K, int bits, float* galpha, void* stream);
int dgq_adaround_reg_blocks(int64_t numel);
int dgq_adaround_reg_fwd(const float* alpha, int64_t numel, float b, float* partial, void* stream);
int dgq_adaround_reg_bwd(const float* alpha, int64_t numel, float b, const float* g, float* galpha, void* stream);

#ifdef __cplusplus
}
#endif
#endif
```

Measured before the change: 118.4 steps/s.

## Software-pipeline attention key loop, interleaving softmax math between score MFMAs

Adds a pipelined variant of the bf16 attention stats and PV kernels. It computes the next key tile's scores while the current tile's softmax or quantisation math is placed into slots between the MFMA instructions using sched_barrier-guarded fill callbacks. The PV kernel gets an extra LDS ring stage so a further tile can be prefetched. The goal is to hide exp2/max VALU latency behind matrix-core work. The cost is higher register pressure and a larger LDS ring, and the path is on by default for wide non-int8 attention, with an env switch to turn it off.

After: 119.1 steps/s (median of 6 runs). No clear change (+0.6%).

```diff
diff --git a/dgq_amd/_lib.py b/dgq_amd/_lib.py
--- a/dgq_amd/_lib.py
+++ b/dgq_amd/_lib.py
@@ -36,6 +36,7 @@
     "dgq_attention_fuses_fakequant": [_i, _i],
     "dgq_attention_workspace_bytes": [_i, _i, _i, _i, _i],
     "dgq_attention_sync_timeouts": [],
+    "dgq_attention_pipelined_calls": [],
     "dgq_minmax_rows_cols": [_vp, _i, _i, _i, _i64, _vp, _vp, _vp, _vp, _vp, _i, _vp],
     "dgq_linear_smallm_batch": [_vp, _i, _i, _i, _i64, _i, _i, _vp, _i, _vp],
     "dgq_quant_act_batch": [_i, _vp, _vp],
diff --git a/dgq_amd/csrc/attn_bf16x3.hip b/dgq_amd/csrc/attn_bf16x3.hip
--- a/dgq_amd/csrc/attn_bf16x3.hip
+++ b/dgq_amd/csrc/attn_bf16x3.hip
@@ -127,7 +127,7 @@
     DGQ_ATTN_PREP_DONE();
 }
 
-template <int D, int NW, int QM, int TPS = 1>
+template <int D, int NW, int QM, int TPS = 1, bool PIPE = false>
 __global__ __launch_bounds__(64 * NW) void attn3_stats_kernel(AttnParams p) {
     using G = Geo<D, QM>;
     constexpr bool QI8 = G::QI8, KS = QM == 3;
@@ -148,7 +148,7 @@
     const uint32_t lds_base = (uint32_t)(uintptr_t)(lptr_t)lds8;
     const int nsp = gridDim.z, i0 = (int)((long)p.NT * blockIdx.z / nsp), i1 = (int)((long)p.NT * (blockIdx.z + 1) / nsp);
 #pragma unroll
-    for (int i = 0; i < ST - 1; ++i)
+    for (int i = 0; i < (PIPE ? ST : ST - 1); ++i)
 #pragma unroll
         for (int j = 0; j < TPS; ++j)
             issue_image<NP, NW>(img_lane + (int64_t)min(i0 + TPS * i + j, i1 - 1) * p.img_bytes, lds_base + i * SB + j * TB, wid);
@@ -172,38 +172,21 @@
     }
     const float sl2 = p.scale * LOG2E * qt.x * dk;
     float mraw = -INFINITY, l = 0.0f, m2raw = -INFINITY;
-    DGQ_STAMP(3);
-    wait_image<NP, TPS * (ST - 2), NW>(wid);
-    __builtin_amdgcn_s_barrier();
-    DGQ_STAMP(4);
-    int stage = 0, istage = ST - 1;
-    for (int ib = i0; ib < i1; ib += TPS) {
-#pragma unroll
-      for (int jt = 0; jt < TPS; ++jt)
-        issue_image<NP, NW>(img_lane + (int64_t)min(ib + TPS * (ST - 1) + jt, i1 - 1) * p.img_bytes, lds_base + istage * SB + jt * TB, wid);
-#pragma unroll
-      for (int jt = 0; jt < TPS; ++jt) {
-        const int i = ib + jt;
-        const unsigned char* tile_lds = lds8 + stage * SB + jt * TB;
-        const int s0 = i * KT;
-        v16f acc;
-        if constexpr (QI8) acc = score_tile_i8<D, KS>(tile_lds, qc, qt, lane, i == 0 && p.kskip > 0, inv_dk, cq);
-        else if constexpr (QM == 2) acc = score_tile_q1<D>(reinterpret_cast<const unsigned short*>(tile_lds), qf, qt.y, lane);
-        else acc = score_tile<D>(reinterpret_cast<const unsigned short*>(tile_lds), qf, lane);
-        const bool edge = (s0 + KT > p.S) || (s0 < p.skip);
+    auto score = [&](const unsigned char* tile_lds, int i, const auto& fill) -> v16f {
+        if constexpr (QI8) return score_tile_i8<D, KS>(tile_lds, qc, qt, lane, i == 0 && p.kskip > 0, inv_dk, cq);
+        else if constexpr (QM == 2) return score_tile_q1<D>(reinterpret_cast<const unsigned short*>(tile_lds), qf, qt.y, lane, fill);
+        else return score_tile<D>(reinterpret_cast<const unsigned short*>(tile_lds), qf, lane, fill);
+    };
+    static_assert(!(PIPE && QI8), "the pipelined key loop serves the bf16 score forms");
+    constexpr int NM = G::NKK * (QM == 2 ? 3 : 6);
+    auto update_edge = [&](v16f acc, int s0) {
         float tmax = -INFINITY, tmax2 = -INFINITY;
-        if (edge) {
-#pragma unroll
-            for (int r = 0; r < 16; ++r) {
-                const int s = s0 + key_of(r, h32);
-                if (s >= p.S) acc[r] = -INFINITY;
-                tmax = fmaxf(tmax, acc[r]);
-                if (s >= p.skip) tmax2 = fmaxf(tmax2, acc[r]);
-            }
-        } else {
-#pragma unroll
-            for (int r = 0; r < 16; ++r) tmax = fmaxf(tmax, acc[r]);
-            tmax2 = tmax;
+#pragma unroll
+        for (int r = 0; r < 16; ++r) {
+            const int s = s0 + key_of(r, h32);
+            if (s >= p.S) acc[r] = -INFINITY;
+            tmax = fmaxf(tmax, acc[r]);
+            if (s >= p.skip) tmax2 = fmaxf(tmax2, acc[r]);
         }
         const float mn = fmaxf(mraw, tmax);
         const float nb = (mn == -INFINITY) ? 0.0f : -(mn * sl2);
@@ -217,6 +200,80 @@
         l = l * __builtin_amdgcn_exp2f(fmaf(mraw, sl2, nb)) + (part.x + part.y);
         mraw = mn;
         m2raw = fmaxf(m2raw, tmax2);
+    };
+    constexpr int NA = 10;
+    float u_tmax = 0.0f, u_mn = 0.0f, u_nb = 0.0f;
+    f2 u_part = {0.0f, 0.0f};
+    auto update_atom = [&](const v16f& acc, int a) {
+        if (a == 0) {
+            float tmax = -INFINITY;
+#pragma unroll
+            for (int r = 0; r < 16; ++r) tmax = fmaxf(tmax, acc[r]);
+            u_tmax = tmax;
+            u_mn = fmaxf(mraw, tmax);
+            u_nb = (u_mn == -INFINITY) ? 0.0f : -(u_mn * sl2);
+            u_part = f2{0.0f, 0.0f};
+        } else if (a < NA - 1) {
+            const int r = 2 * (a - 1);
+            const f2 sl2v = {sl2, sl2}, nbv = {u_nb, u_nb};
+            const f2 x = pk_fma(f2{acc[r], acc[r + 1]}, sl2v, nbv);
+            u_part = pk_add(u_part, f2{__builtin_amdgcn_exp2f(x.x), __builtin_amdgcn_exp2f(x.y)});
+        } else {
+            l = l * __builtin_amdgcn_exp2f(fmaf(mraw, sl2, u_nb)) + (u_part.x + u_part.y);
+            mraw = u_mn;
+            m2raw = fmaxf(m2raw, u_tmax);
+        }
+    };
+    DGQ_STAMP(3);
+    wait_image<NP, TPS * (PIPE ? ST - 1 : ST - 2), NW>(wid);
+    __builtin_amdgcn_s_barrier();
+    DGQ_STAMP(4);
+    int stage = 0, istage = ST - 1;
+    if constexpr (PIPE) {
+        v16f acc = score(lds8, i0, NoFill{});
+        for (int ib = i0; ib < i1; ib += TPS) {
+            const int nstage = (stage + 1 == ST) ? 0 : stage + 1;
+#pragma unroll
+            for (int jt = 0; jt < TPS; ++jt) {
+                const int i = ib + jt, s0 = i * KT;
+                const unsigned char* next_lds = lds8 + stage * SB + (jt + 1) * TB;
+                if (jt == TPS - 1) {
+                    wait_image<NP, TPS * (ST - 2), NW>(wid);
+                    asm volatile("s_waitcnt lgkmcnt(0)" ::: "memory");
+                    __builtin_amdgcn_s_barrier();
+#pragma unroll
+                    for (int j = 0; j < TPS; ++j)
+                        issue_image<NP, NW>(img_lane + (int64_t)min(ib + TPS * ST + j, i1 - 1) * p.img_bytes, lds_base + stage * SB + j * TB, wid);
+                    next_lds = lds8 + nstage * SB;
+                }
+                const bool edge = (s0 + KT > p.S) || (s0 < p.skip);
+                v16f accn;
+                if (!edge) {
+                    auto atom = [&](int a) { update_atom(acc, a); };
+                    accn = score(next_lds, i + 1, SlotFill<NM, NA, decltype(atom)>{atom});
+                } else {
+                    update_edge(acc, s0);
+                    accn = score(next_lds, i + 1, NoFill{});
+                }
+                acc = accn;
+            }
+            stage = nstage;
+        }
+    } else
+    for (int ib = i0; ib < i1; ib += TPS) {
+#pragma unroll
+      for (int jt = 0; jt < TPS; ++jt)
+        issue_image<NP, NW>(img_lane + (int64_t)min(ib + TPS * (ST - 1) + jt, i1 - 1) * p.img_bytes, lds_base + istage * SB + jt * TB, wid);
+#pragma unroll
+      for (int jt = 0; jt < TPS; ++jt) {
+        const int i = ib + jt;
+        const int s0 = i * KT;
+        const v16f acc = score(lds8 + stage * SB + jt * TB, i, NoFill{});
+        if ((s0 + KT > p.S) || (s0 < p.skip)) update_edge(acc, s0);
+        else {
+#pragma unroll
+            for (int a = 0; a < NA; ++a) update_atom(acc, a);
+        }
       }
         wait_image<NP, TPS * (ST - 2), NW>(wid);
         __builtin_amdgcn_s_barrier();
@@ -311,11 +368,11 @@
     }
 }
 
-template <int D, bool UNIFORM, int NW, int QM, bool VINT, int TPS = 1>
+template <int D, bool UNIFORM, int NW, int QM, bool VINT, int TPS = 1, bool PIPE = false>
 __global__ __launch_bounds__(64 * NW) void attn3_pv_kernel(AttnParams p) {
     using G = Geo<D, QM, VINT>;
     constexpr bool QI8 = G::QI8, KS = QM == 3;
-    constexpr int ST = TPS > 1 ? 2 : G::PV_STAGES, NP = G::IMG_PIECES, TB = G::IMG_BYTES, SB = TPS * TB;
+    constexpr int ST = (TPS > 1 ? 2 : G::PV_STAGES) + (PIPE ? 1 : 0), NP = G::IMG_PIECES, TB = G::IMG_BYTES, SB = TPS * TB;
     extern __shared__ __attribute__((aligned(16))) unsigned char lds8[];
     const int tid = threadIdx.x, lane = tid & 63, wid = tid >> 6, h32 = lane >> 5;
     DGQ_DIAG_DECL
@@ -384,22 +441,39 @@
     asm volatile("s_waitcnt vmcnt(0)" ::: "memory");
     __builtin_amdgcn_s_barrier();
     DGQ_STAMP(4);
-    int stage = 0, istage = ST - 1;
-    for (int ib = i0; ib < i1; ib += TPS) {
-#pragma unroll
-      for (int jt = 0; jt < TPS; ++jt)
-        issue_image<NP, NW>(img_lane + (int64_t)min(ib + TPS * (ST - 1) + jt, i1 - 1) * G::IMG_BYTES, lds_base + istage * SB + jt * TB, wid);
-#pragma unroll
-      for (int jt = 0; jt < TPS; ++jt) {
-        const int i = ib + jt;
-        const int s0 = i * KT;
-        const unsigned short* kbc = reinterpret_cast<const unsigned short*>(lds8 + stage * SB + jt * TB);
-        const unsigned short* vtc = kbc + G::K_ELEMS;
-        v16f acc;
-        if constexpr (QI8) acc = score_tile_i8<D, KS>(lds8 + stage * SB + jt * TB, qc, qt, lane, i == 0 && p.kskip > 0, inv_dk, cq);
-        else if constexpr (QM == 2) acc = score_tile_q1<D>(kbc, qf, qt.y, lane);
-        else acc = score_tile<D>(kbc, qf, lane);
-        const bool edge = (s0 + KT > p.S) || (s0 < p.skip);
+    auto score = [&](const unsigned char* tile_lds, int i, const auto& fill) -> v16f {
+        if constexpr (QI8) return score_tile_i8<D, KS>(tile_lds, qc, qt, lane, i == 0 && p.kskip > 0, inv_dk, cq);
+        else if constexpr (QM == 2) return score_tile_q1<D>(reinterpret_cast<const unsigned short*>(tile_lds), qf, qt.y, lane, fill);
+        else return score_tile<D>(reinterpret_cast<const unsigned short*>(tile_lds), qf, lane, fill);
+    };
+    static_assert(!(PIPE && QI8), "the pipelined key loop serves the bf16 score forms");
+    constexpr int NM = G::NKK * (QM == 2 ? 3 : 6);
+    auto quant_atom = [&](const v16f& acc, unsigned (&w)[8], f2& ps2, int j) {
+        const int r = 2 * j;
+        if constexpr (UNIFORM) {
+            const int cmaxu_i = MAGIC_I + (int)p.qmax;
+            const f2 sl2v = {sl2, sl2}, na0v = {-a0, -a0}, magic = {MAGIC, MAGIC}, nmagic = {-MAGIC, -MAGIC};
+            const f2 a = pk_fma(f2{acc[r], acc[r + 1]}, sl2v, na0v);
+            const f2 y = pk_add(f2{__builtin_amdgcn_exp2f(a.x), __builtin_amdgcn_exp2f(a.y)}, magic);
+            const f2 c = pk_add(f2{__int_as_float(min(__float_as_int(y.x), cmaxu_i)), __int_as_float(min(__float_as_int(y.y), cmaxu_i))}, nmagic);
+            if constexpr (VINT && !G::VONES) ps2 = pk_add(ps2, c);
+            w[j] = __builtin_amdgcn_perm(__float_as_uint(c.y), __float_as_uint(c.x), 0x07060302u);
+        } else {
+            const f2 nsl2v = {nsl2, nsl2}, a0m = {a0, a0}, magic = {MAGIC, MAGIC};
+            const f2 y = pk_add(pk_fma(f2{acc[r], acc[r + 1]}, nsl2v, a0m), magic);
+            const int c0 = min(max(__float_as_int(y.x), MAGIC_I), cmax_i), c1 = min(max(__float_as_int(y.y), MAGIC_I), cmax_i);
+            if constexpr (VINT && !G::VONES) psum += __int_as_float(0x3F800000 - (c0 << 23)) + __int_as_float(0x3F800000 - (c1 << 23));
+            const unsigned pair = __builtin_amdgcn_perm((unsigned)c1, (unsigned)c0, 0x05040100u);
+            w[j] = (unsigned)(__mul24((int)pair, -128) + 0x3F803F80);
+        }
+    };
+    auto quant_pack = [&](const unsigned (&w)[8], const f2& ps2, bf16x8 (&pf)[2]) {
+        if constexpr (UNIFORM && VINT && !G::VONES) psum += ps2.x + ps2.y;
+        pf[0] = __builtin_bit_cast(bf16x8, make_uint4(w[0], w[1], w[2], w[3]));
+        pf[1] = __builtin_bit_cast(bf16x8, make_uint4(w[4], w[5], w[6], w[7]));
+    };
+    auto quantise_tile = [&](v16f acc, int s0, bf16x8 (&pf)[2], auto edge_tag) {
+        constexpr bool EDGE = decltype(edge_tag)::value;
         auto quantise = [&](auto edge_tag) {
             constexpr bool EDGE = decltype(edge_tag)::value;
 #pragma unroll
@@ -426,46 +500,14 @@
                 if constexpr (VINT && !G::VONES) psum += ph;
             }
         };
-        bf16x8 pf[2];
-        if (UNIFORM && !edge) {
-            const int cmaxu_i = MAGIC_I + (int)p.qmax;
-            const f2 sl2v = {sl2, sl2}, na0v = {-a0, -a0}, magic = {MAGIC, MAGIC}, nmagic = {-MAGIC, -MAGIC};
+        if constexpr (!EDGE) {
+            unsigned w[8];
             f2 ps2 = {0.0f, 0.0f};
-            unsigned w[8];
-#pragma unroll
-            for (int r = 0; r < 16; r += 2) {
-                const f2 a = pk_fma(f2{acc[r], acc[r + 1]}, sl2v, na0v);
-                const f2 y = pk_add(f2{__builtin_amdgcn_exp2f(a.x), __builtin_amdgcn_exp2f(a.y)}, magic);
-                const f2 c = pk_add(f2{__int_as_float(min(__float_as_int(y.x), cmaxu_i)), __int_as_float(min(__float_as_int(y.y), cmaxu_i))}, nmagic);
-                if constexpr (VINT && !G::VONES) ps2 = pk_add(ps2, c);
-                w[r >> 1] = __builtin_amdgcn_perm(__float_as_uint(c.y), __float_as_uint(c.x), 0x07060302u);
-            }
-            if constexpr (VINT && !G::VONES) psum += ps2.x + ps2.y;
-            pf[0] = __builtin_bit_cast(bf16x8, make_uint4(w[0], w[1], w[2], w[3]));
-            pf[1] = __builtin_bit_cast(bf16x8, make_uint4(w[4], w[5], w[6], w[7]));
-        } else if (!UNIFORM && !edge) {
-            int ci[16];
-            const f2 nsl2v = {nsl2, nsl2}, a0m = {a0, a0}, magic = {MAGIC, MAGIC};
-#pragma unroll
-            for (int r = 0; r < 16; r += 2) {
-                const f2 y = pk_add(pk_fma(f2{acc[r], acc[r + 1]}, nsl2v, a0m), magic);
-                ci[r] = min(max(__float_as_int(y.x), MAGIC_I), cmax_i);
-                ci[r + 1] = min(max(__float_as_int(y.y), MAGIC_I), cmax_i);
-                if constexpr (VINT && !G::VONES) psum += __int_as_float(0x3F800000 - (ci[r] << 23)) + __int_as_float(0x3F800000 - (ci[r + 1] << 23));
-            }
-#pragma unroll
-            for (int ks = 0; ks < 2; ++ks) {
-                unsigned w[4];
-#pragma unroll
-                for (int i = 0; i < 4; ++i) {
-                    const unsigned pair = __builtin_amdgcn_perm((unsigned)ci[8 * ks + 2 * i + 1], (unsigned)ci[8 * ks + 2 * i], 0x05040100u);
-                    w[i] = (unsigned)(__mul24((int)pair, -128) + 0x3F803F80);
-                }
-                pf[ks] = __builtin_bit_cast(bf16x8, make_uint4(w[0], w[1], w[2], w[3]));
-            }
+#pragma unroll
+            for (int j = 0; j < 8; ++j) quant_atom(acc, w, ps2, j);
+            quant_pack(w, ps2, pf);
         } else {
-            if (edge) quantise(std::true_type{});
-            else quantise(std::false_type{});
+            quantise(edge_tag);
 #pragma unroll
             for (int ks = 0; ks < 2; ++ks) {
 #define PK(i) ((__float_as_uint(acc[8 * ks + 2 * (i)]) >> 16) | (__float_as_uint(acc[8 * ks + 2 * (i) + 1]) & 0xFFFF0000u))
@@ -473,6 +515,8 @@
 #undef PK
             }
         }
+    };
+    auto pv_tile = [&](const unsigned short* vtc, const bf16x8 (&pf)[2]) {
 #pragma unroll
         for (int j = 0; j < G::NDT; ++j) {
             const unsigned short* vp = vtc + (j * 32 + (lane & 31)) * G::VLD + 8 * h32;
@@ -488,6 +532,59 @@
                 oacc[j] = __builtin_amdgcn_mfma_f32_32x32x16_bf16(vh, pf[ks], oacc[j], 0, 0, 0);
             }
         }
+    };
+    int stage = 0, istage = ST - 1;
+    if constexpr (PIPE) {
+        v16f acc = score(lds8, i0, NoFill{});
+        for (int ib = i0; ib < i1; ib += TPS) {
+            const int nstage = (stage + 1 == ST) ? 0 : stage + 1;
+#pragma unroll
+            for (int jt = 0; jt < TPS; ++jt) {
+                const int i = ib + jt, s0 = i * KT;
+                const unsigned char* next_lds = lds8 + stage * SB + (jt + 1) * TB;
+                if (jt == TPS - 1) {
+                    wait_image<NP, TPS * (ST - 3), NW>(wid);
+                    asm volatile("s_waitcnt lgkmcnt(0)" ::: "memory");
+                    __builtin_amdgcn_s_barrier();
+#pragma unroll
+                    for (int j = 0; j < TPS; ++j)
+                        issue_image<NP, NW>(img_lane + (int64_t)min(ib + TPS * (ST - 1) + j, i1 - 1) * G::IMG_BYTES, lds_base + istage * SB + j * TB, wid);
+                    next_lds = lds8 + nstage * SB;
+                }
+                const bool edge = (s0 + KT > p.S) || (s0 < p.skip);
+                v16f accn;
+                bf16x8 pf[2];
+                if (!edge) {
+                    unsigned w[8];
+                    f2 ps2 = {0.0f, 0.0f};
+                    auto atom = [&](int j) { quant_atom(acc, w, ps2, j); };
+                    accn = score(next_lds, i + 1, SlotFill<NM, 8, decltype(atom)>{atom});
+                    quant_pack(w, ps2, pf);
+                } else {
+                    quantise_tile(acc, s0, pf, std::true_type{});
+                    accn = score(next_lds, i + 1, NoFill{});
+                }
+                pv_tile(reinterpret_cast<const unsigned short*>(lds8 + stage * SB + jt * TB) + G::K_ELEMS, pf);
+                acc = accn;
+            }
+            stage = nstage;
+            istage = (istage + 1 == ST) ? 0 : istage + 1;
+        }
+    } else
+    for (int ib = i0; ib < i1; ib += TPS) {
+#pragma unroll
+      for (int jt = 0; jt < TPS; ++jt)
+        issue_image<NP, NW>(img_lane + (int64_t)min(ib + TPS * (ST - 1) + jt, i1 - 1) * G::IMG_BYTES, lds_base + istage * SB + jt * TB, wid);
+#pragma unroll
+      for (int jt = 0; jt < TPS; ++jt) {
+        const int i = ib + jt;
+        const int s0 = i * KT;
+        const unsigned char* tile_lds = lds8 + stage * SB + jt * TB;
+        const v16f acc = score(tile_lds, i, NoFill{});
+        bf16x8 pf[2];
+        if ((s0 + KT > p.S) || (s0 < p.skip)) quantise_tile(acc, s0, pf, std::true_type{});
+        else quantise_tile(acc, s0, pf, std::false_type{});
+        pv_tile(reinterpret_cast<const unsigned short*>(tile_lds) + G::K_ELEMS, pf);
       }
         wait_image<NP, TPS * (ST - 2), NW>(wid);
         __builtin_amdgcn_s_barrier();
@@ -581,6 +678,9 @@
     DGQ_DIAG_FLUSH(attn, NW, wid, lane);
 }
 
+static std::atomic<int> attn_pipelined_calls{0};
+extern "C" int dgq_attention_pipelined_calls(void) { return attn_pipelined_calls.load(std::memory_order_relaxed); }
+
 template <int D, int QM, bool VINT>
 static int launch_attn3(AttnParams p, const void* q_raw, unsigned char* planes, float* qfq, hipStream_t st) {
     using G = Geo<D, QM, VINT>;
@@ -595,7 +695,11 @@
     constexpr int pv_lds = pv_ring > pv_scratch ? pv_ring : pv_scratch;
     constexpr int TPS_P = (2 * DGQ_ATTN_TPS_PV * G::IMG_BYTES <= 160 * 1024) ? DGQ_ATTN_TPS_PV : 2;
     constexpr int pv2_ring = D <= 64 ? 2 * TPS_P * G::IMG_BYTES : 0, pv2_lds = pv2_ring > pv_scratch ? pv2_ring : pv_scratch;
-    static_assert(stats_lds <= 160 * 1024 && pv_lds <= 160 * 1024 && stats2_lds <= 160 * 1024 && pv2_lds <= 160 * 1024, "LDS ring too large");
+    constexpr bool PV2P = D <= 64 && 3 * TPS_P * G::IMG_BYTES <= 160 * 1024;
+    constexpr int pvp_ring = D <= 64 ? (G::PV_STAGES + 1) * G::IMG_BYTES : 0, pvp_lds = pvp_ring > pv_scratch ? pvp_ring : pv_scratch;
+    constexpr int pv2p_ring = PV2P ? 3 * TPS_P * G::IMG_BYTES : 0, pv2p_lds = pv2p_ring > pv_scratch ? pv2p_ring : pv_scratch;
+    static_assert(stats_lds <= 160 * 1024 && pv_lds <= 160 * 1024 && stats2_lds <= 160 * 1024 && pv2_lds <= 160 * 1024 && pvp_lds <= 160 * 1024 &&
+                  pv2p_lds <= 160 * 1024, "LDS ring too large");
     static std::atomic<bool> attr_set[64];
     int dev = 0;
     (void)hipGetDevice(&dev);
@@ -610,6 +714,16 @@
             (void)hipFuncSetAttribute(reinterpret_cast<const void*>(&attn3_pv_kernel<D, false, 8, QM, VINT>), hipFuncAttributeMaxDynamicSharedMemorySize, pv_lds);
             (void)hipFuncSetAttribute(reinterpret_cast<const void*>(&attn3_pv_kernel<D, true, 8, QM, VINT, TPS_P>), hipFuncAttributeMaxDynamicSharedMemorySize, pv2_lds);
             (void)hipFuncSetAttribute(reinterpret_cast<const void*>(&attn3_pv_kernel<D, false, 8, QM, VINT, TPS_P>), hipFuncAttributeMaxDynamicSharedMemorySize, pv2_lds);
+            if constexpr (!QI8) {
+            (void)hipFuncSetAttribute(reinterpret_cast<const void*>(&attn3_stats_kernel<D, 8, QM, 1, true>), hipFuncAttributeMaxDynamicSharedMemorySize, stats_lds);
+            (void)hipFuncSetAttribute(reinterpret_cast<const void*>(&attn3_stats_kernel<D, 8, QM, TPS_S, true>), hipFuncAttributeMaxDynamicSharedMemorySize, stats2_lds);
+            (void)hipFuncSetAttribute(reinterpret_cast<const void*>(&attn3_pv_kernel<D, true, 8, QM, VINT, 1, true>), hipFuncAttributeMaxDynamicSharedMemorySize, pvp_lds);
+            (void)hipFuncSetAttribute(reinterpret_cast<const void*>(&attn3_pv_kernel<D, false, 8, QM, VINT, 1, true>), hipFuncAttributeMaxDynamicSharedMemorySize, pvp_lds);
+            }
+            if constexpr (PV2P && !QI8) {
+                (void)hipFuncSetAttribute(reinterpret_cast<const void*>(&attn3_pv_kernel<D, true, 8, QM, VINT, TPS_P, true>), hipFuncAttributeMaxDynamicSharedMemorySize, pv2p_lds);
+                (void)hipFuncSetAttribute(reinterpret_cast<const void*>(&attn3_pv_kernel<D, false, 8, QM, VINT, TPS_P, true>), hipFuncAttributeMaxDynamicSharedMemorySize, pv2p_lds);
+            }
         }
         if (dev >= 0 && dev < 64) attr_set[dev].store(true, std::memory_order_release);
     }
@@ -655,7 +769,26 @@
     const long split_below = se ? atol(se) : 448L;
     const long nblk4 = (long)((p.T + 127) / 128) * p.B * p.H;
     const int nsp = (!wide && nblk4 < split_below && p.NT >= 8 && D % 4 == 0) ? 2 : 1;
-    if (wide) {
+    const char* pe = getenv("DGQ_ATTN_PIPE");
+    const bool pipe = !QI8 && !(pe != nullptr && pe[0] == '0');
+    if (wide && pipe) {
+        if constexpr (D <= 64 && !QI8) {
+            dim3 grid((p.T + 255) / 256, p.B * p.H), block(512);
+            if (p.NT >= 4 * TPS_S && p.NT % TPS_S == 0) hipLaunchKernelGGL((attn3_stats_kernel<D, 8, QM, TPS_S, true>), grid, block, stats2_lds, st, p);
+            else hipLaunchKernelGGL((attn3_stats_kernel<D, 8, QM, 1, true>), grid, block, stats_lds, st, p);
+            bool two = false;
+            if constexpr (PV2P) {
+                two = p.NT >= 4 * TPS_P && p.NT % TPS_P == 0;
+                if (two && p.mode == 3) hipLaunchKernelGGL((attn3_pv_kernel<D, true, 8, QM, VINT, TPS_P, true>), grid, block, pv2p_lds, st, p);
+                else if (two) hipLaunchKernelGGL((attn3_pv_kernel<D, false, 8, QM, VINT, TPS_P, true>), grid, block, pv2p_lds, st, p);
+            }
+            if (!two) {
+                if (p.mode == 3) hipLaunchKernelGGL((attn3_pv_kernel<D, true, 8, QM, VINT, 1, true>), grid, block, pvp_lds, st, p);
+                else hipLaunchKernelGGL((attn3_pv_kernel<D, false, 8, QM, VINT, 1, true>), grid, block, pvp_lds, st, p);
+            }
+            attn_pipelined_calls.fetch_add(1, std::memory_order_relaxed);
+        }
+    } else if (wide) {
         if constexpr (D <= 64) {
             dim3 grid((p.T + 255) / 256, p.B * p.H), block(512);
             if (p.NT >= 4 * TPS_S && p.NT % TPS_S == 0) hipLaunchKernelGGL((attn3_stats_kernel<D, 8, QM, TPS_S>), grid, block, stats2_lds, st, p);
diff --git a/dgq_amd/csrc/attn_bf16x3_dev.h b/dgq_amd/csrc/attn_bf16x3_dev.h
--- a/dgq_amd/csrc/attn_bf16x3_dev.h
+++ b/dgq_amd/csrc/attn_bf16x3_dev.h
@@ -218,8 +218,23 @@
     }
 }
 
-template <int D>
-__device__ __forceinline__ v16f score_tile(const unsigned short* kb, const bf16x8 (&qf)[3][Geo<D>::NKK], int lane) {
+struct NoFill {
+    __device__ __forceinline__ void operator()(int) const {}
+};
+template <int NM, int NA, typename ATOM>
+struct SlotFill {
+    ATOM& atom;
+    __device__ __forceinline__ void operator()(int n) const {
+        __builtin_amdgcn_sched_barrier(0x104);
+#pragma unroll
+        for (int a = 0; a < NA; ++a)
+            if (((a + 1) * NM - 1) / NA == n) atom(a);
+        __builtin_amdgcn_sched_barrier(0x104);
+    }
+};
+
+template <int D, typename FILL = NoFill>
+__device__ __forceinline__ v16f score_tile(const unsigned short* kb, const bf16x8 (&qf)[3][Geo<D>::NKK], int lane, const FILL& fill = FILL{}) {
     using G = Geo<D>;
     constexpr bool DUAL = D >= 64;
     v16f acc, acc2;
@@ -234,18 +249,30 @@
         const bf16x8 kl = *reinterpret_cast<const bf16x8*>(kp + 2 * PL + 16 * kk);
         if (DUAL) {
             acc2 = __builtin_amdgcn_mfma_f32_32x32x16_bf16(kl, qf[0][kk], acc2, 0, 0, 0);
+            fill(6 * kk);
             acc = __builtin_amdgcn_mfma_f32_32x32x16_bf16(km, qf[0][kk], acc, 0, 0, 0);
+            fill(6 * kk + 1);
             acc2 = __builtin_amdgcn_mfma_f32_32x32x16_bf16(kh, qf[2][kk], acc2, 0, 0, 0);
+            fill(6 * kk + 2);
             acc = __builtin_amdgcn_mfma_f32_32x32x16_bf16(kh, qf[1][kk], acc, 0, 0, 0);
+            fill(6 * kk + 3);
             acc2 = __builtin_amdgcn_mfma_f32_32x32x16_bf16(km, qf[1][kk], acc2, 0, 0, 0);
+            fill(6 * kk + 4);
             acc = __builtin_amdgcn_mfma_f32_32x32x16_bf16(kh, qf[0][kk], acc, 0, 0, 0);
+            fill(6 * kk + 5);
         } else {
             acc = __builtin_amdgcn_mfma_f32_32x32x16_bf16(kl, qf[0][kk], acc, 0, 0, 0);
+            fill(6 * kk);
             acc = __builtin_amdgcn_mfma_f32_32x32x16_bf16(kh, qf[2][kk], acc, 0, 0, 0);
+            fill(6 * kk + 1);
             acc = __builtin_amdgcn_mfma_f32_32x32x16_bf16(km, qf[1][kk], acc, 0, 0, 0);
+            fill(6 * kk + 2);
             acc = __builtin_amdgcn_mfma_f32_32x32x16_bf16(km, qf[0][kk], acc, 0, 0, 0);
+            fill(6 * kk + 3);
             acc = __builtin_amdgcn_mfma_f32_32x32x16_bf16(kh, qf[1][kk], acc, 0, 0, 0);
+            fill(6 * kk + 4);
             acc = __builtin_amdgcn_mfma_f32_32x32x16_bf16(kh, qf[0][kk], acc, 0, 0, 0);
+            fill(6 * kk + 5);
         }
     }
     if (DUAL) {
@@ -324,8 +351,8 @@
         qf[0][D / 16] = __builtin_bit_cast(bf16x8, make_uint4((unsigned)zh | ((unsigned)zm << 16), (unsigned)zl, 0u, 0u));
 }
 
-template <int D>
-__device__ __forceinline__ v16f score_tile_q1(const unsigned short* kb, const bf16x8 (&qf)[3][Geo<D>::NKK], float zmul, int lane) {
+template <int D, typename FILL = NoFill>
+__device__ __forceinline__ v16f score_tile_q1(const unsigned short* kb, const bf16x8 (&qf)[3][Geo<D>::NKK], float zmul, int lane, const FILL& fill = FILL{}) {
     using G = Geo<D, 2, false>;
     v16f acc;
 #pragma unroll
@@ -338,8 +365,11 @@
         const bf16x8 km = *reinterpret_cast<const bf16x8*>(kp + PL + 16 * kk);
         const bf16x8 kl = *reinterpret_cast<const bf16x8*>(kp + 2 * PL + 16 * kk);
         acc = __builtin_amdgcn_mfma_f32_32x32x16_bf16(kl, qf[0][kk], acc, 0, 0, 0);
+        fill(3 * kk);
         acc = __builtin_amdgcn_mfma_f32_32x32x16_bf16(km, qf[0][kk], acc, 0, 0, 0);
+        fill(3 * kk + 1);
         acc = __builtin_amdgcn_mfma_f32_32x32x16_bf16(kh, qf[0][kk], acc, 0, 0, 0);
+        fill(3 * kk + 2);
     }
     if constexpr (!G::FOLDZ) {
         const float* tv = reinterpret_cast<const float*>(kb + 3 * PL);
diff --git a/dgq_amd/ops.py b/dgq_amd/ops.py
--- a/dgq_amd/ops.py
+++ b/dgq_amd/ops.py
@@ -1052,6 +1052,10 @@
 attention_f32 = attention
 
 
+def attention_pipelined_calls():
+    return _lib.load().dgq_attention_pipelined_calls()
+
+
 def attention_sync_timeouts():
     n = _lib.load().dgq_attention_sync_timeouts()
     if n < 0:
diff --git a/include/dgq_hip.h b/include/dgq_hip.h
--- a/include/dgq_hip.h
+++ b/include/dgq_hip.h
@@ -154,6 +154,7 @@
 int dgq_attention_fuses_fakequant(int D, int mode);
 size_t dgq_attention_workspace_bytes(int B, int H, int T, int S, int D);
 int dgq_attention_sync_timeouts(void);
+int dgq_attention_pipelined_calls(void);
 
 typedef struct dgq_smallm_problem {
     const void* wpacked;
```
